# eMWu94/ReMo3D

Measured on AMD Instinct MI355X. Metric: measurement points/sec (3D benchmark model), higher is better.
Workload: dtype f64

## Files before the change

include/remo3d_hip_debug.h:

```cpp
#ifndef REMO3D_HIP_DEBUG_H
#define REMO3D_HIP_DEBUG_H

#include "remo3d_hip.h"

#ifdef __cplusplus
extern "C" {
#endif

int remo_debug_stream(remo_ctx_t *ctx, int64_t bytes, double *read_gbs, double *copy_gbs);
int remo_debug_clock(remo_ctx_t *ctx, double *gfma_per_wave);
int remo_debug_cache_gather(remo_ctx_t *ctx, int64_t bytes, double *gbs);
int remo_debug_device(remo_ctx_t *ctx, int64_t *out8);
int remo_debug_xcc(remo_ctx_t *ctx, int32_t *out, int32_t nblocks);


int remo_debug_patch_phases(remo_ctx_t *ctx, remo_batch_t *batch, int32_t fp32 , double *out16);

int remo_debug_patch_phases_p(remo_ctx_t *ctx, remo_batch_t *batch, int32_t fp32, double *out16);

int remo_debug_grid_barrier(remo_ctx_t *ctx, int32_t nblocks, int32_t nbar, double *out3);

int remo_debug_sens_timing(remo_ctx_t *ctx, double *out2);
int remo_debug_sens_group_timing(remo_ctx_t *ctx, double *out4);
int remo_debug_field_timing(remo_ctx_t *ctx, double *out2);
int remo_debug_point_location(remo_ctx_t *ctx);
int remo_debug_direction_bytes(remo_ctx_t *ctx);
int remo_debug_direction_forms(remo_ctx_t *ctx, int64_t n, int64_t nv, int32_t k, int32_t grid, int32_t step, double tol2, const double *r,
                               const float *p, const double *z, const double *dinv, const double *part_even, const double *part_odd,
                               int32_t nb_rz, const double *scal48, float *p_flat, float *p_row, double *scal_flat, double *scal_row);
int remo_debug_product(remo_ctx_t *ctx, int32_t slots, int64_t cap, int64_t nx, const int32_t *xrp, const int32_t *xc, const double *xv,
                       int64_t ny, const int32_t *yrp, const int32_t *yc, const double *yv, int32_t *crp, int32_t *cc, double *cv,
                       int32_t *flags);
int remo_debug_vector_heads(remo_ctx_t *ctx, int32_t on, double *out8);
int remo_debug_secondary_timing(remo_ctx_t *ctx, double *ms);
int remo_debug_pairs_timing(remo_ctx_t *ctx, double *out2);
int remo_debug_pair_groups_timing(remo_ctx_t *ctx, double *out4);

int remo_debug_tune(int32_t key, int32_t value);

#ifdef __cplusplus
}
#endif
#endif
```

remo3d_amd/_lib.py:

```python
from __future__ import annotations

import ctypes as C
import os

import numpy as np

_HERE = os.path.dirname(os.path.abspath(__file__))
LIB_PATH = os.environ.get("REMO_LIB") or os.path.join(_HERE, "libremo3d_hip.so")
REMO_MAX_RHS = 8


class RemoMesh(C.Structure):
    _fields_ = [("dim", C.c_int32), ("n_nodes", C.c_int64), ("coords", C.POINTER(C.c_double)),
                ("n_elems", C.c_int64), ("conn", C.POINTER(C.c_int32)), ("mat", C.POINTER(C.c_int32)),
                ("n_bfacets", C.c_int64), ("bconn", C.POINTER(C.c_int32)), ("bdirichlet", C.POINTER(C.c_uint8))]


class RemoOpts(C.Structure):
    _fields_ = [("preconditioner", C.c_int32), ("condense", C.c_int32), ("maxsteps", C.c_int32),
                ("check_every", C.c_int32), ("rtol", C.c_double), ("time_kernels", C.c_int32),
                ("coarse_degree", C.c_int32), ("coarse_ratio", C.c_int32), ("precision", C.c_int32), ("inner_digits", C.c_int32),
                ("serialize_solves", C.c_int32), ("op", C.c_int32), ("coarse", C.c_int32), ("assemble", C.c_int32), ("quadrature", C.c_int32)]


class RemoStats(C.Structure):
    _fields_ = [("n_dof", C.c_int64), ("n_free", C.c_int64), ("nnz", C.c_int64), ("n_edges", C.c_int64),
                ("n_faces", C.c_int64), ("n_rhs", C.c_int32), ("max_iterations", C.c_int32),
                ("iterations", C.c_int32 * REMO_MAX_RHS), ("relres", C.c_double * REMO_MAX_RHS),
                ("ms_symbolic", C.c_double), ("ms_h2d", C.c_double), ("ms_assemble", C.c_double),
                ("ms_solve", C.c_double), ("ms_eval", C.c_double), ("ms_total", C.c_double),
                ("spmv_ms", C.c_double), ("spmv_launches", C.c_int64), ("spmv_bytes", C.c_double),
                ("pcg_steps", C.c_int64), ("spmv_ms_raw", C.c_double), ("event_overhead_ms", C.c_double),
                ("refinement_cycles", C.c_int64), ("op_used", C.c_int32), ("coarse_used", C.c_int32),
                ("assembled", C.c_int32), ("patch_rounds", C.c_int32)]

    def as_dict(self):
        d = {}
        for name, _ in self._fields_:
            v = getattr(self, name)
            d[name] = list(v) if hasattr(v, "__len__") else v
        return d


class RemoJob(C.Structure):
    _dp, _ip = C.POINTER(C.c_double), C.POINTER(C.c_int32)
    _fields_ = [("size", C.c_uint32), ("tensor", C.c_int32), ("n_mat", C.c_int32), ("sigma", _dp),
                ("n_rhs", C.c_int32), ("src_ptr", _ip), ("src_p", _dp), ("src_I", _dp),
                ("eval_ptr", _ip), ("eval_p", _dp), ("u_out", _dp),
                ("n_fun", C.c_int32), ("fun_rhs", _ip), ("fun_ptr", _ip), ("fun_p", _dp), ("fun_w", _dp), ("J_out", _dp), ("dJ_out", _dp),
                ("n_group", C.c_int32), ("group", _ip), ("dJg_out", _dp),
                ("warm", C.c_void_p),
                ("n_pts", C.c_int32), ("pts", _dp), ("n_frhs", C.c_int32), ("field_rhs", _ip), ("u_f", _dp), ("grad_f", _dp), ("J_f", _dp),
                ("elem_f", _ip)]


class RemoJobSecondary(C.Structure):
    _fields_ = RemoJob._fields_ + [("secondary", C.c_int32), ("sec_quad", C.c_int32), ("sec_radius", C.c_double),
                                   ("sec_sigma0", C.POINTER(C.c_double))]


class RemoJobError(C.Structure):
    _fields_ = RemoJobSecondary._fields_ + [("err", C.c_int32), ("err_n_group", C.c_int32), ("err_group", C.POINTER(C.c_int32)),
                                            ("err_out", C.POINTER(C.c_double)), ("errg_out", C.POINTER(C.c_double))]


class RemoJobPairs(C.Structure):
    _fields_ = RemoJobError._fields_ + [("n_pair", C.c_int32), ("pair_reserved", C.c_int32), ("pair_a", C.POINTER(C.c_int32)),
                                        ("pair_b", C.POINTER(C.c_int32)), ("dP_out", C.POINTER(C.c_double))]


class RemoJobPairGroups(C.Structure):
    _fields_ = RemoJobPairs._fields_ + [("pair_n_group", C.c_int32), ("pair_group_reserved", C.c_int32), ("pair_group", C.POINTER(C.c_int32)),
                                        ("dPg_out", C.POINTER(C.c_double))]


EXPORTS = ["remo_abi_version", "remo_opts_default", "remo_ctx_create", "remo_ctx_destroy", "remo_last_error",
           "remo_solve_batch", "remo_solve_batch_tensor", "remo_solve_batch_sens", "remo_solve_batch_sens_tensor", "remo_solve_batch_sens_groups", "remo_solve_batch_sens_groups_tensor",
           "remo_solve_batch_field", "remo_solve_batch_field_tensor", "remo_batch_field", "remo_host_field_element",
           "remo_warm_create", "remo_warm_destroy", "remo_warm_clear", "remo_warm_info", "remo_solve_batch_sens_warm", "remo_solve_batch_sens_warm_tensor", "remo_batch_create", "remo_batch_create_tensor", "remo_batch_run", "remo_batch_fetch", "remo_batch_destroy",
           "remo_batch_eval", "remo_batch_get_system", "remo_batch_get_vectors", "remo_batch_apply_coarse", "remo_batch_spmv",
           "remo_host_element_matrix", "remo_host_element_matrix_tensor", "remo_host_sens_element", "remo_host_factor_error", "remo_host_symbolic",
           "remo_solve_job", "remo_batch_create_job", "remo_host_point_shapes", "remo_host_secondary_element", "remo_host_error_facet", "remo_host_pair_element"]
DEBUG_EXPORTS = ["remo_debug_stream", "remo_debug_clock", "remo_debug_device", "remo_debug_cache_gather", "remo_debug_xcc", "remo_debug_tune", "remo_debug_patch_phases", "remo_debug_patch_phases_p", "remo_debug_grid_barrier", "remo_debug_sens_timing", "remo_debug_sens_group_timing", "remo_debug_field_timing", "remo_debug_point_location", "remo_debug_secondary_timing", "remo_debug_direction_bytes", "remo_debug_pairs_timing", "remo_debug_pair_groups_timing",
                 "remo_debug_direction_forms", "remo_debug_vector_heads", "remo_debug_product"]

JOB_HEAD = ["n_mat", "sigma", "n_rhs", "src_ptr", "src_p", "src_I", "eval_ptr", "eval_p"]
_SENS = ["u_out", "n_fun", "fun_rhs", "fun_ptr", "fun_p", "fun_w"]
LEGACY_MEMBERS = {"": ["u_out"],
                  "_sens": _SENS + ["J_out", "dJ_out"],
                  "_sens_warm": _SENS + ["J_out", "dJ_out", "warm"],
                  "_sens_groups": _SENS + ["n_group", "group", "J_out", "dJ_out", "dJg_out"],
                  "_field": ["u_out", "n_pts", "pts", "n_frhs", "field_rhs", "u_f", "grad_f", "J_f", "elem_f"]}


def legacy_args(job, kind=None):
    return [getattr(job, name) for name in JOB_HEAD + (LEGACY_MEMBERS[kind] if kind is not None else [])]


_lib = None


def load():
    global _lib
    if _lib is not None:
        return _lib
    if not os.path.exists(LIB_PATH):
        raise ImportError(f"{LIB_PATH} is missing: build it with `make -C remo3d_amd/csrc` "
                          "(or __graft_entry__.build()); remo3d_amd has no CPU fallback")
    L = C.CDLL(LIB_PATH)
    dp, ip, i64p, u8p = C.POINTER(C.c_double), C.POINTER(C.c_int32), C.POINTER(C.c_int64), C.POINTER(C.c_uint8)
    vp = C.c_void_p
    L.remo_abi_version.restype = C.c_int
    L.remo_opts_default.argtypes = [C.POINTER(RemoOpts)]
    L.remo_ctx_create.restype = vp
    L.remo_ctx_create.argtypes = [C.c_int]
    L.remo_ctx_destroy.argtypes = [vp]
    L.remo_last_error.restype = C.c_char_p
    L.remo_last_error.argtypes = [vp]
    member = dict(RemoJob._fields_)
    batch_args = [vp, C.POINTER(RemoMesh)] + [member[name] for name in JOB_HEAD]
    for kind, names in LEGACY_MEMBERS.items():
        for entry in (getattr(L, "remo_solve_batch" + kind), getattr(L, "remo_solve_batch" + kind + "_tensor")):
            entry.restype = C.c_int
            entry.argtypes = batch_args + [member[name] for name in names] + [C.POINTER(RemoOpts), C.POINTER(RemoStats)]
    L.remo_warm_create.restype = vp
    L.remo_warm_create.argtypes = [C.c_int]
    L.remo_warm_destroy.restype = None
    L.remo_warm_destroy.argtypes = [vp]
    L.remo_warm_clear.restype = None
    L.remo_warm_clear.argtypes = [vp]
    L.remo_warm_info.restype = C.c_int
    L.remo_warm_info.argtypes = [vp, i64p, ip, i64p, ip]
    L.remo_solve_job.restype = C.c_int
    L.remo_solve_job.argtypes = [vp, C.POINTER(RemoMesh), vp, C.POINTER(RemoOpts), C.POINTER(RemoStats)]
    L.remo_batch_create_job.restype = C.c_int
    L.remo_batch_create_job.argtypes = [vp, C.POINTER(RemoMesh), vp, C.POINTER(vp)]
    L.remo_host_point_shapes.restype = C.c_int
    L.remo_host_point_shapes.argtypes = [C.c_int32, dp, dp, dp]
    L.remo_batch_field.restype = C.c_int
    L.remo_batch_field.argtypes = [vp, vp, C.c_int32, C.c_int32, dp, dp, dp, dp, ip]
    L.remo_host_field_element.restype = C.c_int
    L.remo_host_field_element.argtypes = [C.c_int32, dp, dp, C.c_double, dp, dp, dp]
    L.remo_debug_field_timing.restype = C.c_int
    L.remo_debug_field_timing.argtypes = [vp, dp]
    L.remo_debug_point_location.restype = C.c_int
    L.remo_debug_point_location.argtypes = [vp]
    L.remo_debug_direction_bytes.restype = C.c_int
    L.remo_debug_direction_bytes.argtypes = [vp]
    L.remo_host_secondary_element.restype = C.c_int
    L.remo_host_secondary_element.argtypes = [C.c_int32, dp, dp, C.c_double, C.c_double, C.c_double, dp, C.c_int32, dp]
    L.remo_host_error_facet.restype = C.c_int
    L.remo_host_error_facet.argtypes = [C.c_int32, C.c_int32, dp, dp, C.c_double, dp, dp, dp, C.c_double, dp, dp]
    L.remo_debug_secondary_timing.restype = C.c_int
    L.remo_debug_secondary_timing.argtypes = [vp, dp]
    L.remo_debug_sens_group_timing.restype = C.c_int
    L.remo_debug_sens_group_timing.argtypes = [vp, dp]
    L.remo_host_pair_element.restype = C.c_int
    L.remo_host_pair_element.argtypes = [C.c_int32, dp, C.c_int32, C.c_int32, dp, C.c_int32, ip, ip, dp]
    L.remo_debug_pairs_timing.restype = C.c_int
    L.remo_debug_pairs_timing.argtypes = [vp, dp]
    L.remo_debug_pair_groups_timing.restype = C.c_int
    L.remo_debug_pair_groups_timing.argtypes = [vp, dp]
    L.remo_host_sens_element.restype = C.c_int
    L.remo_host_sens_element.argtypes = [C.c_int32, dp, C.c_int32, dp, dp, dp]
    L.remo_debug_sens_timing.restype = C.c_int
    L.remo_debug_sens_timing.argtypes = [vp, dp]
    L.remo_batch_create.restype = C.c_int
    L.remo_batch_create.argtypes = batch_args + [C.POINTER(vp)]
    L.remo_batch_create_tensor.restype = C.c_int
    L.remo_batch_create_tensor.argtypes = batch_args + [C.POINTER(vp)]
    L.remo_batch_run.restype = C.c_int
    L.remo_batch_run.argtypes = [vp, vp, C.POINTER(RemoOpts), C.POINTER(RemoStats)]
    L.remo_batch_fetch.restype = C.c_int
    L.remo_batch_fetch.argtypes = [vp, vp, dp]
    L.remo_batch_destroy.argtypes = [vp, vp]
    L.remo_batch_eval.restype = C.c_int
    L.remo_batch_eval.argtypes = [vp, vp, C.c_int32, C.c_int32, dp, dp]
    L.remo_batch_get_system.restype = C.c_int
    L.remo_batch_get_system.argtypes = [vp, vp, ip, ip, dp, dp, ip]
    L.remo_batch_get_vectors.restype = C.c_int
    L.remo_batch_get_vectors.argtypes = [vp, vp, dp, dp, ip]
    L.remo_batch_apply_coarse.restype = C.c_int
    L.remo_batch_apply_coarse.argtypes = [vp, vp, C.c_int32, dp, dp, C.c_int32, i64p]
    L.remo_debug_patch_phases.restype = C.c_int
    L.remo_debug_patch_phases.argtypes = [vp, vp, C.c_int32, dp]
    L.remo_debug_patch_phases_p.restype = C.c_int
    L.remo_debug_patch_phases_p.argtypes = [vp, vp, C.c_int32, dp]
    L.remo_debug_grid_barrier.restype = C.c_int
    L.remo_debug_grid_barrier.argtypes = [vp, C.c_int32, C.c_int32, dp]
    L.remo_debug_xcc.restype = C.c_int
    L.remo_debug_xcc.argtypes = [vp, ip, C.c_int32]
    L.remo_debug_cache_gather.restype = C.c_int
    L.remo_debug_cache_gather.argtypes = [vp, C.c_int64, dp]
    L.remo_debug_device.restype = C.c_int
    L.remo_debug_device.argtypes = [vp, i64p]
    L.remo_debug_clock.restype = C.c_int
    L.remo_debug_clock.argtypes = [vp, dp]
    L.remo_debug_stream.restype = C.c_int
    L.remo_debug_stream.argtypes = [vp, C.c_int64, dp, dp]
    L.remo_batch_spmv.restype = C.c_int
    L.remo_batch_spmv.argtypes = [vp, vp, C.c_int32, dp, dp, C.c_int32, dp]
    L.remo_host_element_matrix.restype = C.c_int
    L.remo_host_element_matrix.argtypes = [C.c_int32, dp, C.c_double, dp]
    L.remo_host_element_matrix_tensor.restype = C.c_int
    L.remo_host_element_matrix_tensor.argtypes = [C.c_int32, dp, dp, dp]
    L.remo_host_factor_error.restype = C.c_double
    L.remo_host_symbolic.restype = C.c_int
    L.remo_host_symbolic.argtypes = [C.POINTER(RemoMesh), C.c_int32, i64p, ip, ip, ip]
    L.remo_debug_tune.restype = C.c_int
    L.remo_debug_tune.argtypes = [C.c_int32, C.c_int32]
    fp = C.POINTER(C.c_float)
    if hasattr(L, "remo_debug_direction_forms"):
        L.remo_debug_direction_forms.restype = C.c_int
        L.remo_debug_direction_forms.argtypes = [vp, C.c_int64, C.c_int64, C.c_int32, C.c_int32, C.c_int32, C.c_double, dp, fp, dp, dp, dp, dp,
                                                 C.c_int32, dp, fp, fp, dp, dp]
        L.remo_debug_vector_heads.restype = C.c_int
        L.remo_debug_vector_heads.argtypes = [vp, C.c_int32, dp]
    if hasattr(L, "remo_debug_product"):
        L.remo_debug_product.restype = C.c_int
        L.remo_debug_product.argtypes = [vp, C.c_int32, C.c_int64, C.c_int64, ip, ip, dp, C.c_int64, ip, ip, dp, ip, ip, dp, ip]
    _lib = L
    return L


def ptr(a, t):
    return a.ctypes.data_as(C.POINTER(t))


def mesh_struct(mesh):
    coords = np.ascontiguousarray(mesh.coords, dtype=np.float64)
    conn = np.ascontiguousarray(mesh.conn, dtype=np.int32)
    mat = np.ascontiguousarray(mesh.mat, dtype=np.int32)
    bconn = np.ascontiguousarray(mesh.bconn, dtype=np.int32).reshape(-1, mesh.dim)
    bdir = np.ascontiguousarray(mesh.bdirichlet, dtype=np.uint8)
    m = RemoMesh(int(mesh.dim), coords.shape[0], ptr(coords, C.c_double), conn.shape[0], ptr(conn, C.c_int32),
                 ptr(mat, C.c_int32), bconn.shape[0], ptr(bconn, C.c_int32), ptr(bdir, C.c_uint8))
    return m, (coords, conn, mat, bconn, bdir)
```

remo3d_amd/csrc/amg.h:

```cpp
#pragma once
#include <hip/hip_runtime.h>
#include <stdint.h>

#include <string>

#include "symbolic_gpu.h"

namespace remo {

constexpr int kAmgMaxLevels = 8;
constexpr int kAmgDenseMax = 64;

template <class T> struct AmgLevelT {
    int64_t n = 0, nnz = 0, nnz_p = 0;
    const int32_t *rowptr = nullptr, *col = nullptr;
    const T *val = nullptr, *dinv = nullptr;
    const int32_t *p_rowptr = nullptr, *p_col = nullptr;
    const T *p_val = nullptr;
    const int32_t *r_rowptr = nullptr, *r_col = nullptr;
    const T *r_val = nullptr;
    double omega = 0.0;
    T *r = nullptr, *z = nullptr, *z2 = nullptr, *t = nullptr;
};

template <class T> struct AmgT {
    int levels = 0;
    AmgLevelT<T> lev[kAmgMaxLevels];
    const T *inv = nullptr;
    int launches = 0;
    int kmax = 0;
};

bool amg_setup(Arena &ar, hipStream_t s, int dim, int64_t nv, const int32_t *rowptr, const int32_t *col, const double *val, int kmax,
               AmgT<double> &out, std::string &why);
void amg_to_float(Arena &ar, hipStream_t s, const AmgT<double> &in, int kmax, AmgT<float> &out);

void amg_debug_product(hipStream_t s, int slots, int64_t cap, int64_t nx, const int32_t *xrp, const int32_t *xc, const double *xv, int64_t ny,
                       const int32_t *yrp, const int32_t *yc, const double *yv, int32_t *crp, int32_t *cc, double *cv, int32_t *flags);

template <class T, class TR> void launch_amg_cycle(const AmgT<T> &H, int k, int step, const TR *r, TR *cz, double *part, int nblocks, const double *scal,
                                                   hipStream_t s);

}
```

remo3d_amd/csrc/amg.hip:

```cpp
#include <hip/hip_runtime.h>
#include <limits.h>

#include <rocprim/device/device_scan.hpp>

#include <atomic>
#include <cmath>
#include <cstdio>
#include <cstdlib>
#include <cstring>
#include <stdexcept>
#include <string>
#include <vector>

#include "amg.h"
#include "remo_internal.h"
#include "wave_util.h"
#include "kutil.h"

namespace remo {
namespace {

__device__ __forceinline__ void wave_sync() {
    __builtin_amdgcn_fence(__ATOMIC_ACQ_REL, "wavefront");
    __builtin_amdgcn_wave_barrier();
}

__device__ __forceinline__ bool amg_done(const double *scal, int step) {
    if (!scal) return false;
    const int d = reinterpret_cast<const int *>(scal + kDoneSlot)[0];
    return d != 0 && d <= step;
}

template <int PASS>
__global__ void __launch_bounds__(256) k_block_copy(int64_t nv, const int32_t *__restrict__ rowptr, const int32_t *__restrict__ col,
                                                    const double *__restrict__ val, int32_t *__restrict__ cnt, const int32_t *__restrict__ orp,
                                                    int32_t *__restrict__ oc, double *__restrict__ ov) {
    const int64_t row = int64_t(blockIdx.x) * blockDim.x + threadIdx.x;
    if (row >= nv) return;
    const int32_t rs = rowptr[row], re = rowptr[row + 1];
    if (PASS == 0) {
        cnt[row] = lower_bound_i32(col, rs, re, int32_t(nv)) - rs;
    } else {
        const int32_t at = orp[row], len = orp[row + 1] - at;
        for (int32_t e = 0; e < len; ++e) { oc[at + e] = col[rs + e]; ov[at + e] = val[rs + e]; }
    }
}

__global__ void __launch_bounds__(256) k_level_diag(int64_t n, const int32_t *__restrict__ rowptr, const int32_t *__restrict__ col,
                                                    const double *__restrict__ val, double *__restrict__ dinv, unsigned long long *bound_bits,
                                                    int32_t *flag) {
    double m = 0.0;
    const int64_t row = int64_t(blockIdx.x) * blockDim.x + threadIdx.x;
    if (row < n) {
        double s = 0.0, d = 0.0;
        for (int32_t p = rowptr[row]; p < rowptr[row + 1]; ++p) {
            s += fabs(val[p]);
            if (col[p] == row) d = val[p];
        }
        if (!(d > 0.0)) { atomicOr(flag, 1); d = 1.0; }
        dinv[row] = 1.0 / d;
        m = s / d;
    }
#pragma unroll
    for (int off = 32; off > 0; off >>= 1) m = fmax(m, __shfl_xor(m, off, 64));
    if ((threadIdx.x & 63) == 0) atomicMax(bound_bits, (unsigned long long)__double_as_longlong(m));
}

constexpr uint64_t kTupMask = (uint64_t(1) << 62) - 1;

__device__ __forceinline__ uint32_t hash_u32(uint32_t x) {
    x ^= x >> 16; x *= 0x7feb352du; x ^= x >> 15; x *= 0x846ca68bu; x ^= x >> 16;
    return x;
}

__global__ void __launch_bounds__(256) k_mis_init(int64_t n, uint64_t *__restrict__ tup) {
    const int64_t i = int64_t(blockIdx.x) * blockDim.x + threadIdx.x;
    if (i < n) tup[i] = (uint64_t(1) << 62) | (uint64_t(hash_u32(uint32_t(i)) >> 2) << 32) | uint64_t(uint32_t(i));
}

__global__ void __launch_bounds__(256) k_mis_max(int64_t n, const int32_t *__restrict__ rowptr, const int32_t *__restrict__ col,
                                                 const uint64_t *__restrict__ tup, uint64_t *__restrict__ m1) {
    const int64_t i = int64_t(blockIdx.x) * blockDim.x + threadIdx.x;
    if (i >= n) return;
    uint64_t m = tup[i];
    for (int32_t p = rowptr[i]; p < rowptr[i + 1]; ++p) { const uint64_t t = tup[col[p]]; m = t > m ? t : m; }
    m1[i] = m;
}

__global__ void __launch_bounds__(256) k_mis_update(int64_t n, const int32_t *__restrict__ rowptr, const int32_t *__restrict__ col,
                                                    uint64_t *__restrict__ tup, const uint64_t *__restrict__ m1) {
    const int64_t i = int64_t(blockIdx.x) * blockDim.x + threadIdx.x;
    if (i >= n) return;
    const uint64_t t = tup[i];
    if ((t >> 62) != 1) return;
    uint64_t m = m1[i];
    for (int32_t p = rowptr[i]; p < rowptr[i + 1]; ++p) { const uint64_t v = m1[col[p]]; m = v > m ? v : m; }
    if (m == t) tup[i] = (uint64_t(2) << 62) | (t & kTupMask);
    else if ((m >> 62) == 2) tup[i] = t & kTupMask;
}

__global__ void __launch_bounds__(256) k_mis_finish(int64_t n, const int32_t *__restrict__ rowptr, const int32_t *__restrict__ col,
                                                    const uint64_t *__restrict__ tup, uint64_t *__restrict__ out) {
    const int64_t i = int64_t(blockIdx.x) * blockDim.x + threadIdx.x;
    if (i >= n) return;
    const uint64_t t = tup[i];
    uint64_t r = t;
    if ((t >> 62) == 1) {
        bool top = true;
        for (int32_t p = rowptr[i]; p < rowptr[i + 1]; ++p) {
            const uint64_t v = tup[col[p]];
            if ((v >> 62) == 1 && v > t) top = false;
        }
        r = top ? ((uint64_t(2) << 62) | (t & kTupMask)) : (t & kTupMask);
    }
    out[i] = r;
}

__global__ void __launch_bounds__(256) k_mis_flags(int64_t n, const uint64_t *__restrict__ tup, int32_t *__restrict__ isroot) {
    const int64_t i = int64_t(blockIdx.x) * blockDim.x + threadIdx.x;
    if (i < n) isroot[i] = (tup[i] >> 62) == 2 ? 1 : 0;
}

__global__ void __launch_bounds__(256) k_agg_near(int64_t n, const int32_t *__restrict__ rowptr, const int32_t *__restrict__ col,
                                                  const uint64_t *__restrict__ tup, const int32_t *__restrict__ id, int32_t *__restrict__ agg) {
    const int64_t i = int64_t(blockIdx.x) * blockDim.x + threadIdx.x;
    if (i >= n) return;
    if ((tup[i] >> 62) == 2) { agg[i] = id[i]; return; }
    uint64_t best = 0;
    int32_t bj = -1;
    for (int32_t p = rowptr[i]; p < rowptr[i + 1]; ++p) {
        const int32_t j = col[p];
        const uint64_t t = tup[j];
        if ((t >> 62) == 2 && t > best) { best = t; bj = j; }
    }
    agg[i] = bj >= 0 ? id[bj] : -1;
}

__global__ void __launch_bounds__(256) k_agg_far(int64_t n, const int32_t *__restrict__ rowptr, const int32_t *__restrict__ col,
                                                 const double *__restrict__ val, const int32_t *__restrict__ agg_in, int32_t *__restrict__ agg_out) {
    const int64_t i = int64_t(blockIdx.x) * blockDim.x + threadIdx.x;
    if (i >= n) return;
    int32_t a = agg_in[i];
    if (a < 0) {
        double w = -1.0;
        for (int32_t p = rowptr[i]; p < rowptr[i + 1]; ++p) {
            const int32_t j = col[p];
            if (j == i) continue;
            const int32_t aj = agg_in[j];
            const double v = fabs(val[p]);
            if (aj >= 0 && v > w) { w = v; a = aj; }
        }
    }
    agg_out[i] = a;
}

__global__ void __launch_bounds__(256) k_smoothing_factor(int64_t n, const int32_t *__restrict__ rowptr, const int32_t *__restrict__ col,
                                                          const double *__restrict__ val, const double *__restrict__ dinv, const unsigned long long *bound_bits,
                                                          double *__restrict__ sval, const int32_t *__restrict__ agg, int32_t *__restrict__ p0rp,
                                                          int32_t *__restrict__ p0c, double *__restrict__ p0v) {
    const int64_t i = int64_t(blockIdx.x) * blockDim.x + threadIdx.x;
    if (i > n) return;
    p0rp[i] = int32_t(i);
    if (i == n) return;
    const double f = 4.0 / (3.0 * __longlong_as_double((long long)bound_bits[0])) * dinv[i];
    for (int32_t p = rowptr[i]; p < rowptr[i + 1]; ++p) sval[p] = (col[p] == i ? 1.0 : 0.0) - f * val[p];
    const int32_t a = agg[i];
    p0c[i] = a >= 0 ? a : 0;
    p0v[i] = a >= 0 ? 1.0 : 0.0;
}

template <int PASS, int SLOTS>
__global__ void __launch_bounds__(256) k_spgemm(int64_t nx, const int32_t *__restrict__ xrp, const int32_t *__restrict__ xc, const double *__restrict__ xv,
                                                const int32_t *__restrict__ yrp, const int32_t *__restrict__ yc, const double *__restrict__ yv,
                                                int32_t *__restrict__ cnt, const int32_t *__restrict__ crp, int32_t *__restrict__ cc,
                                                double *__restrict__ cv, int32_t *flag) {
    __shared__ int32_t keys[4][SLOTS];
    __shared__ int32_t list[4][SLOTS];
    constexpr int kTerms = SLOTS < 512 ? 512 : 1024;
    __shared__ double terms[4][PASS == 1 ? kTerms : 1];
    __shared__ int32_t pstart[4][PASS == 1 ? 64 : 1], pys[4][PASS == 1 ? 64 : 1];
    __shared__ double pxv[4][PASS == 1 ? 64 : 1];
    const int wave = threadIdx.x >> 6, lane = threadIdx.x & 63;
    const int64_t row = int64_t(blockIdx.x) * 4 + wave;
    if (row >= nx) return;
    int32_t *K = keys[wave], *L = list[wave];
    for (int sl = lane; sl < SLOTS; sl += 64) K[sl] = INT_MAX;
    wave_sync();
    const int32_t xs = xrp[row], xe = xrp[row + 1];
    bool overflow = false;
    for (int32_t p = xs + lane; p < xe; p += 64) {
        const int32_t k = xc[p];
        const int32_t ye = yrp[k + 1];
        for (int32_t q = yrp[k]; q < ye; ++q) {
            const int32_t j = yc[q];
            uint32_t h = ((uint32_t(j) * 2654435761u) >> 16) & (SLOTS - 1);
            bool placed = false;
            for (int probe = 0; probe < SLOTS; ++probe) {
                const int32_t old = atomicCAS(&K[h], INT_MAX, j);
                if (old == INT_MAX || old == j) { placed = true; break; }
                h = (h + 1) & (SLOTS - 1);
            }
            overflow |= !placed;
        }
    }
    wave_sync();
    int c = 0;
    for (int base = 0; base < SLOTS; base += 64) {
        const int32_t v = K[base + lane];
        const bool occ = v != INT_MAX;
        const uint64_t bal = __builtin_amdgcn_ballot_w64(occ);
        if (occ) L[c + __builtin_popcountll(bal & ((uint64_t(1) << lane) - 1))] = v;
        c += __builtin_popcountll(bal);
    }
    if (__builtin_amdgcn_ballot_w64(overflow) != 0 || c > SLOTS / 2) {
        if (lane == 0) atomicOr(flag, 1);
        c = 0;
    }
    if (PASS == 0) {
        if (lane == 0) cnt[row] = c;
        return;
    }
    if (c == 0) return;
    int m = 64;
    while (m < c) m <<= 1;
    for (int t = c + lane; t < m; t += 64) L[t] = INT_MAX;
    wave_sync();
    for (int size = 2; size <= m; size <<= 1)
        for (int stride = size >> 1; stride > 0; stride >>= 1) {
            for (int t = lane; t < m / 2; t += 64) {
                const int lo = 2 * t - (t & (stride - 1));
                const int hi = lo + stride;
                const bool up = (lo & size) == 0;
                const int32_t a = L[lo], b = L[hi];
                if ((a > b) == up) { L[lo] = b; L[hi] = a; }
            }
            wave_sync();
        }
    const int64_t off = crp[row];
    const int room = int(crp[row + 1] - crp[row]);
    if (c > room) c = room;
    if (c <= 0) return;
    double *V = terms[wave];
    int32_t *PS = pstart[wave], *PY = pys[wave];
    double *PX = pxv[wave];
    constexpr int NACC = SLOTS / 128;
    double acc[NACC];
#pragma unroll
    for (int a = 0; a < NACC; ++a) acc[a] = 0.0;
    const int npmax = kTerms / c < 64 ? kTerms / c : 64;
    for (int i = lane; i < c * npmax; i += 64) V[i] = 0.0;
    for (int32_t p0 = xs; p0 < xe; p0 += npmax) {
        const int np = (xe - p0 < npmax) ? int(xe - p0) : npmax;
        int32_t ys = 0, len = 0;
        double xval = 0.0;
        if (lane < np) {
            const int32_t k = xc[p0 + lane];
            xval = xv[p0 + lane];
            ys = yrp[k];
            len = yrp[k + 1] - ys;
        }
        int32_t incl = len;
#pragma unroll
        for (int off = 1; off < 64; off <<= 1) {
            const int32_t up = __shfl_up(incl, off, 64);
            if (lane >= off) incl += up;
        }
        const int32_t total = __shfl(incl, 63, 64);
        if (lane < np) { PS[lane] = incl - len; PY[lane] = ys; PX[lane] = xval; }
        wave_sync();
        for (int32_t idx = lane; idx < total; idx += 64) {
            int lo = 1, hi = np;
            while (lo < hi) {
                const int mid = (lo + hi) >> 1;
                if (PS[mid] <= idx) lo = mid + 1; else hi = mid;
            }
            const int pp = lo - 1;
            const int32_t q = PY[pp] + (idx - PS[pp]);
            const int32_t j = yc[q];
            const double yval = yv[q];
            const int t = lower_bound_i32(L, 0, c, j);
            if (t < c && L[t] == j) V[pp * c + t] = PX[pp] * yval;
        }
        wave_sync();
#pragma unroll
        for (int a = 0; a < NACC; ++a) {
            const int t = lane + 64 * a;
            if (t < c)
                for (int pp = 0; pp < np; ++pp) { acc[a] += V[pp * c + t]; V[pp * c + t] = 0.0; }
        }
    }
#pragma unroll
    for (int a = 0; a < NACC; ++a) {
        const int t = lane + 64 * a;
        if (t < c) { cc[off + t] = L[t]; cv[off + t] = acc[a]; }
    }
}

__global__ void __launch_bounds__(256) k_clamp_rowptr(int64_t n, int32_t *__restrict__ rowptr, int32_t capacity, int32_t *flag) {
    const int64_t i = int64_t(blockIdx.x) * blockDim.x + threadIdx.x;
    if (i > n) return;
    const int32_t v = rowptr[i];
    if (v > capacity) { rowptr[i] = capacity; if (i == n) atomicOr(flag, 2); }
}

__global__ void __launch_bounds__(256) k_tr_count(int64_t n, const int32_t *__restrict__ rowptr, const int32_t *__restrict__ col, int32_t *__restrict__ cnt) {
    const int64_t i = int64_t(blockIdx.x) * blockDim.x + threadIdx.x;
    if (i >= n) return;
    for (int32_t p = rowptr[i]; p < rowptr[i + 1]; ++p) atomicAdd(&cnt[col[p]], 1);
}
__global__ void __launch_bounds__(256) k_tr_fill(int64_t n, const int32_t *__restrict__ rowptr, const int32_t *__restrict__ col, const double *__restrict__ val,
                                                 const int32_t *__restrict__ rrp, int32_t *__restrict__ cursor, int32_t *__restrict__ rc, double *__restrict__ rv) {
    const int64_t i = int64_t(blockIdx.x) * blockDim.x + threadIdx.x;
    if (i >= n) return;
    for (int32_t p = rowptr[i]; p < rowptr[i + 1]; ++p) {
        const int32_t c = col[p];
        const int32_t at = rrp[c] + atomicAdd(&cursor[c], 1);
        rc[at] = int32_t(i);
        rv[at] = val[p];
    }
}
constexpr int kTrMax = 512, kTrMaxLong = 4096;
template <int MINLEN, int MAXLEN, int WAVES>
__global__ void __launch_bounds__(64 * WAVES) k_tr_sort(int64_t nr, const int32_t *__restrict__ rrp, int32_t *__restrict__ rc, double *__restrict__ rv, int32_t *flag) {
    __shared__ int32_t keys[WAVES][MAXLEN];
    __shared__ double vals[WAVES][MAXLEN];
    const int wave = threadIdx.x >> 6, lane = threadIdx.x & 63;
    const int64_t row = int64_t(blockIdx.x) * WAVES + wave;
    if (row >= nr) return;
    const int32_t rs = rrp[row], len = rrp[row + 1] - rs;
    if (len <= 1 || len <= MINLEN) return;
    if (len > MAXLEN) { if (lane == 0 && MAXLEN == kTrMaxLong) atomicOr(flag, 4); return; }
    int32_t *K = keys[wave];
    double *V = vals[wave];
    int m = 64;
    while (m < len) m <<= 1;
    for (int t = lane; t < m; t += 64) { K[t] = t < len ? rc[rs + t] : INT_MAX; V[t] = t < len ? rv[rs + t] : 0.0; }
    wave_sync();
    for (int size = 2; size <= m; size <<= 1)
        for (int stride = size >> 1; stride > 0; stride >>= 1) {
            for (int t = lane; t < m / 2; t += 64) {
                const int lo = 2 * t - (t & (stride - 1));
                const int hi = lo + stride;
                const bool up = (lo & size) == 0;
                const int32_t a = K[lo], b = K[hi];
                if ((a > b) == up) { K[lo] = b; K[hi] = a; const double x = V[lo]; V[lo] = V[hi]; V[hi] = x; }
            }
            wave_sync();
        }
    for (int t = lane; t < len; t += 64) { rc[rs + t] = K[t]; rv[rs + t] = V[t]; }
}

__global__ void __launch_bounds__(256) k_dense_inverse(int n, const int32_t *__restrict__ rowptr, const int32_t *__restrict__ col,
                                                       const double *__restrict__ val, double *__restrict__ inv, int32_t *flag) {
    __shared__ double a[kAmgDenseMax * kAmgDenseMax];
    const int tid = threadIdx.x;
    for (int e = tid; e < n * n; e += 256) a[e] = 0.0;
    __syncthreads();
    for (int i = tid; i < n; i += 256)
        for (int32_t p = rowptr[i]; p < rowptr[i + 1]; ++p) a[i * n + col[p]] = val[p];
    __syncthreads();
    for (int p = 0; p < n; ++p) {
        const double piv = a[p * n + p];
        if (!(piv > 0.0)) { if (tid == 0) atomicOr(flag, 2); return; }
        const double ip = 1.0 / piv;
        __syncthreads();
        for (int j = tid; j < n; j += 256)
            if (j != p) a[p * n + j] *= ip;
        __syncthreads();
        for (int e = tid; e < n * n; e += 256) {
            const int i = e / n, j = e - i * n;
            if (i != p && j != p) a[e] -= a[i * n + p] * a[p * n + j];
        }
        __syncthreads();
        for (int i = tid; i < n; i += 256)
            a[i * n + p] = (i == p) ? ip : -a[i * n + p] * ip;
        __syncthreads();
    }
    for (int e = tid; e < n * n; e += 256) inv[e] = a[e];
}

template <class S, class D> __global__ void __launch_bounds__(256) k_convert(int64_t n, const S *__restrict__ src, D *__restrict__ dst) {
    const int64_t i = int64_t(blockIdx.x) * blockDim.x + threadIdx.x;
    if (i < n) dst[i] = D(src[i]);
}

constexpr int kLpr = 8;

template <class T, int K, bool SCALE, int LPR = kLpr, class TX = T>
__device__ __forceinline__ void row_product(int32_t rs, int32_t re, int sub, const int32_t *__restrict__ col, const T *__restrict__ val,
                                            const T *__restrict__ dinv, const TX *__restrict__ x, T (&acc)[K]) {
#pragma unroll
    for (int c = 0; c < K; ++c) acc[c] = T(0);
    for (int32_t p0 = rs + sub; p0 < re; p0 += 2 * LPR) {
        int32_t j[2];
        T a[2], xv[2][K];
#pragma unroll
        for (int u = 0; u < 2; ++u) {
            const int32_t p = p0 + u * LPR;
            j[u] = -1; a[u] = T(0);
            if (p < re) { j[u] = col[p]; a[u] = val[p]; }
        }
#pragma unroll
        for (int u = 0; u < 2; ++u) {
#pragma unroll
            for (int c = 0; c < K; ++c) xv[u][c] = T(0);
            if (j[u] >= 0) {
                if (SCALE) a[u] *= dinv[j[u]];
                const TX *xr = x + int64_t(j[u]) * K;
#pragma unroll
                for (int c = 0; c < K; ++c) xv[u][c] = T(xr[c]);
            }
        }
#pragma unroll
        for (int u = 0; u < 2; ++u)
#pragma unroll
            for (int c = 0; c < K; ++c) acc[c] += a[u] * xv[u][c];
    }
    TReduce<K, LPR>::run(acc, sub);
}

struct Lane {
    int sub, mycol;
    bool mine;
};
template <int K, int LPR = kLpr> __device__ __forceinline__ Lane lane_of(int tid) {
    int idx[K], own[K];
    Lane l;
    l.sub = tid % LPR;
    towner_init<K, LPR>(idx, own, l.sub);
    l.mycol = idx[0];
    l.mine = own[0] != 0;
    return l;
}

template <class T, int K, class TR = T> __device__ __forceinline__ void op_pre(const AmgLevelT<T> &a, const TR *__restrict__ r, int64_t row, const Lane &ln) {
    T acc[K];
    row_product<T, K, true, kLpr, TR>(a.rowptr[row], a.rowptr[row + 1], ln.sub, a.col, a.val, a.dinv, r, acc);
    if (ln.mine) {
        const int64_t at = row * K + ln.mycol;
        const T w = T(a.omega), ri = T(r[at]);
        a.z[at] = w * a.dinv[row] * ri;
        a.t[at] = ri - w * acc[0];
    }
}
template <class T, int K, int LPR = kLpr> __device__ __forceinline__ void op_restrict(const AmgLevelT<T> &a, T *__restrict__ rn, int64_t row, const Lane &ln) {
    T acc[K];
    row_product<T, K, false, LPR>(a.r_rowptr[row], a.r_rowptr[row + 1], ln.sub, a.r_col, a.r_val, (const T *)nullptr, (const T *)a.t, acc);
    if (ln.mine) rn[row * K + ln.mycol] = acc[0];
}
template <class T, int K> __device__ __forceinline__ void op_prolong(const AmgLevelT<T> &a, const T *__restrict__ zn, int64_t row, const Lane &ln) {
    T acc[K];
    row_product<T, K, false>(a.p_rowptr[row], a.p_rowptr[row + 1], ln.sub, a.p_col, a.p_val, (const T *)nullptr, zn, acc);
    if (ln.mine) a.z[row * K + ln.mycol] += acc[0];
}
template <class T, int K, bool LAST, class TR = T>
__device__ __forceinline__ double op_post(const AmgLevelT<T> &a, const TR *__restrict__ r, TR *__restrict__ zout, int64_t row, const Lane &ln) {
    T acc[K];
    row_product<T, K, false>(a.rowptr[row], a.rowptr[row + 1], ln.sub, a.col, a.val, (const T *)nullptr, (const T *)a.z, acc);
    double dot = 0.0;
    if (ln.mine) {
        const int64_t at = row * K + ln.mycol;
        const TR rr = r[at];
        const T ri = T(rr), di = a.dinv[row];
        const T zn = a.z[at] + T(a.omega) * di * (ri - acc[0]);
        zout[at] = TR(LAST ? zn / di : zn);
        dot = double(rr) * double(zn);
    }
    return dot;
}

constexpr int kRpb = 256 / kLpr;

template <class T, int K, class TR>
__global__ void __launch_bounds__(256) k_amg_pre(AmgLevelT<T> a, const TR *__restrict__ r, const double *scal, int step) {
    if (amg_done(scal, step)) return;
    const Lane ln = lane_of<K>(threadIdx.x);
    const int64_t row = int64_t(blockIdx.x) * kRpb + threadIdx.x / kLpr;
    if (row < a.n) op_pre<T, K, TR>(a, r, row, ln);
}
template <class T, int K>
__global__ void __launch_bounds__(256) k_amg_restrict(AmgLevelT<T> a, int64_t n_next, T *__restrict__ rn, const double *scal, int step) {
    if (amg_done(scal, step)) return;
    const Lane ln = lane_of<K>(threadIdx.x);
    const int64_t row = int64_t(blockIdx.x) * kRpb + threadIdx.x / kLpr;
    if (row < n_next) op_restrict<T, K>(a, rn, row, ln);
}
template <class T, int K>
__global__ void __launch_bounds__(256) k_amg_prolong(AmgLevelT<T> a, const T *__restrict__ zn, const double *scal, int step) {
    if (amg_done(scal, step)) return;
    const Lane ln = lane_of<K>(threadIdx.x);
    const int64_t row = int64_t(blockIdx.x) * kRpb + threadIdx.x / kLpr;
    if (row < a.n) op_prolong<T, K>(a, zn, row, ln);
}
template <class T, int K, bool LAST, int THREADS, class TR>
__global__ void __launch_bounds__(THREADS) k_amg_post(AmgLevelT<T> a, const TR *__restrict__ r, TR *__restrict__ zout,
                                                     double *__restrict__ part, const double *scal, int step) {
    if (amg_done(scal, step)) return;
    const Lane ln = lane_of<K>(threadIdx.x);
    constexpr int RPB = THREADS / kLpr;
    double dot = 0.0;
    for (int64_t row = int64_t(blockIdx.x) * RPB + threadIdx.x / kLpr; row < a.n; row += int64_t(gridDim.x) * RPB)
        dot += op_post<T, K, LAST, TR>(a, r, zout, row, ln);
    if (LAST) {
        constexpr int NW = THREADS / 64;
        __shared__ double smem[NW * K];
        const int lane = threadIdx.x & 63, wave = threadIdx.x >> 6;
#pragma unroll
        for (int k = 0; k < K; ++k) {
            const double x = wave_sum((ln.mine && k == ln.mycol) ? dot : 0.0);
            if (lane == 0) smem[wave * K + k] = x;
        }
        __syncthreads();
        if (threadIdx.x < K) {
            double t = 0.0;
            for (int w = 0; w < NW; ++w) t += smem[w * K + threadIdx.x];
            part[blockIdx.x * K + threadIdx.x] = t;
        }
    }
}

template <class T, int K>
__device__ __forceinline__ void op_dense(int n, const T *__restrict__ inv, const T *__restrict__ r, T *__restrict__ z, int t) {
    const int row = t / K, c = t - row * K;
    T acc = T(0);
    for (int j = 0; j < n; ++j) acc += inv[j * n + row] * r[j * K + c];
    z[t] = acc;
}

constexpr int kTailLevels = 3;
constexpr int kTailRows = 128;
template <class T> struct AmgTailT {
    int levels;
    AmgLevelT<T> up;
    AmgLevelT<T> lev[kTailLevels];
    const T *inv;
};
template <class T, int K>
__global__ void __launch_bounds__(1024) k_amg_tail(AmgTailT<T> A, const double *scal, int step) {
    if (amg_done(scal, step)) return;
    const Lane ln = lane_of<K>(threadIdx.x);
    const int g = threadIdx.x / kLpr, ng = 1024 / kLpr;
    const int L = A.levels;
    {
        const Lane l16 = lane_of<K, 16>(threadIdx.x);
        for (int64_t row = threadIdx.x / 16; row < A.lev[0].n; row += 1024 / 16) op_restrict<T, K, 16>(A.up, A.lev[0].r, row, l16);
        __syncthreads();
    }
    for (int l = 0; l + 1 < L; ++l) {
        const AmgLevelT<T> &a = A.lev[l];
        for (int64_t row = g; row < a.n; row += ng) op_pre<T, K>(a, (const T *)a.r, row, ln);
        __syncthreads();
        const AmgLevelT<T> &b = A.lev[l + 1];
        for (int64_t row = g; row < b.n; row += ng) op_restrict<T, K>(a, b.r, row, ln);
        __syncthreads();
    }
    {
        const AmgLevelT<T> &c = A.lev[L - 1];
        for (int t = threadIdx.x; t < int(c.n) * K; t += 1024) op_dense<T, K>(int(c.n), A.inv, (const T *)c.r, c.z2, t);
        __syncthreads();
    }
    for (int l = L - 2; l >= 0; --l) {
        const AmgLevelT<T> &a = A.lev[l];
        const AmgLevelT<T> &b = A.lev[l + 1];
        for (int64_t row = g; row < a.n; row += ng) op_prolong<T, K>(a, (const T *)b.z2, row, ln);
        __syncthreads();
        for (int64_t row = g; row < a.n; row += ng) (void)op_post<T, K, false>(a, (const T *)a.r, a.z2, row, ln);
        __syncthreads();
    }
}

int grid_rows(int64_t n, int per_block) { return int((n + per_block - 1) / per_block); }

void scan_counts(Arena &ar, hipStream_t s, int64_t n, const int32_t *cnt, int32_t *out) {
    size_t tb = 0;
    HIP_TRY(rocprim::exclusive_scan(nullptr, tb, cnt, out, int32_t(0), size_t(n + 1), rocprim::plus<int32_t>(), s));
    void *tmp = ar.hi<char>(tb + 256);
    HIP_TRY(rocprim::exclusive_scan(tmp, tb, cnt, out, int32_t(0), size_t(n + 1), rocprim::plus<int32_t>(), s));
}

struct Csr {
    int64_t n = 0, nnz = 0;
    int32_t *rowptr = nullptr, *col = nullptr;
    double *val = nullptr;
};

template <int PASS>
void launch_product(int variant, hipStream_t s, const Csr &X, const Csr &Y, int32_t *cnt, const int32_t *crp, int32_t *cc, double *cv, int32_t *d_over) {
    if (variant <= 1)
        hipLaunchKernelGGL((k_spgemm<PASS, 128>), dim3(grid_rows(X.n, 4)), dim3(256), 0, s, X.n, X.rowptr, X.col, X.val, Y.rowptr, Y.col, Y.val, cnt, crp, cc, cv, d_over);
    else
        hipLaunchKernelGGL((k_spgemm<PASS, 512>), dim3(grid_rows(X.n, 4)), dim3(256), 0, s, X.n, X.rowptr, X.col, X.val, Y.rowptr, Y.col, Y.val, cnt, crp, cc, cv, d_over);
}

void spgemm_async(Arena &ar, bool permanent, hipStream_t s, const Csr &X, const Csr &Y, int64_t cap, int variant, int32_t *d_over, Csr &C) {
    if (cap > INT_MAX - 8) cap = INT_MAX - 8;
    C.n = X.n;
    C.nnz = cap;
    C.rowptr = permanent ? ar.lo<int32_t>(size_t(X.n) + 2) : ar.hi<int32_t>(size_t(X.n) + 2);
    int32_t *cnt = ar.hi<int32_t>(size_t(X.n) + 2);
    launch_product<0>(variant, s, X, Y, cnt, nullptr, nullptr, nullptr, d_over);
    scan_counts(ar, s, X.n, cnt, C.rowptr);
    hipLaunchKernelGGL(k_clamp_rowptr, dim3(grid_rows(X.n + 1, 256)), dim3(256), 0, s, X.n, C.rowptr, int32_t(cap), d_over);
    C.col = permanent ? ar.lo<int32_t>(size_t(cap) + 2) : ar.hi<int32_t>(size_t(cap) + 2);
    C.val = permanent ? ar.lo<double>(size_t(cap) + 2) : ar.hi<double>(size_t(cap) + 2);
    launch_product<1>(variant, s, X, Y, nullptr, C.rowptr, C.col, C.val, d_over);
}

std::atomic<int> g_product_hint[2][kAmgMaxLevels][3];
std::atomic<int> g_ap_room[2];
constexpr int kFlagSlots = 64;

int amg_build(Arena &ar, hipStream_t s, int hs, int64_t nv, const int32_t *rowptr, const int32_t *col, const double *val, int kmax, AmgT<double> &H,
              std::string &why) {
    H = AmgT<double>{};
    int32_t *d_flag = ar.lo<int32_t>(kFlagSlots);
    unsigned long long *d_bound = ar.lo<unsigned long long>(kAmgMaxLevels + 1);
    HIP_TRY(hipMemsetAsync(d_flag, 0, sizeof(int32_t) * kFlagSlots, s));
    HIP_TRY(hipMemsetAsync(d_bound, 0, sizeof(unsigned long long) * (kAmgMaxLevels + 1), s));
    int32_t h_flags[kFlagSlots] = {};
    int32_t h_nnz_a[kAmgMaxLevels] = {}, h_nnz_p[kAmgMaxLevels] = {};
    const int32_t *d_nnz_p[kAmgMaxLevels] = {};
    auto check = [&](int upto) -> int {
        int again = 0;
        for (int l = 0; l < upto; ++l)
            for (int p = 0; p < 3; ++p) {
                const int f = h_flags[8 + 3 * l + p];
                if (f == 0) continue;
                if (f & 1) {
                    if (g_product_hint[hs][l][p].load() >= 2) { why = "a product row with more than 256 distinct columns"; return -1; }
                    g_product_hint[hs][l][p].store(2);
                    again = 1;
                }
                if (f & 2) {
                    if (p != 1 || g_ap_room[hs].load() >= 3) { why = "a product outgrew its arrays"; return -1; }
                    g_ap_room[hs].fetch_add(1);
                    again = 1;
                }
            }
        if (again) return 1;
        if (h_flags[0] != 0) {
            why = "setup raised flag " + std::to_string(h_flags[0]) + " (1 diagonal, 2 dense pivot, 4 a row of R beyond the LDS sort)";
            return -1;
        }
        return 0;
    };
    Csr A;
    A.n = nv;
    A.rowptr = ar.lo<int32_t>(size_t(nv) + 2);
    {
        const size_t mark = ar.hi_mark();
        int32_t *cnt = ar.hi<int32_t>(size_t(nv) + 2);
        hipLaunchKernelGGL((k_block_copy<0>), dim3(grid_rows(nv, 256)), dim3(256), 0, s, nv, rowptr, col, val, cnt, (const int32_t *)nullptr,
                           (int32_t *)nullptr, (double *)nullptr);
        scan_counts(ar, s, nv, cnt, A.rowptr);
        int32_t h = 0;
        HIP_TRY(hipMemcpyAsync(&h, A.rowptr + nv, sizeof(int32_t), hipMemcpyDeviceToHost, s));
        HIP_TRY(hipStreamSynchronize(s));
        ar.hi_release(mark);
        if (h <= 0 || h == INT_MAX) { why = "empty vertex block"; return -1; }
        A.nnz = h;
        h_nnz_a[0] = h;
        A.col = ar.lo<int32_t>(size_t(h) + 2);
        A.val = ar.lo<double>(size_t(h) + 2);
        hipLaunchKernelGGL((k_block_copy<1>), dim3(grid_rows(nv, 256)), dim3(256), 0, s, nv, rowptr, col, val, (int32_t *)nullptr,
                           (const int32_t *)A.rowptr, A.col, A.val);
    }
    int L = 0;
    for (;;) {
        AmgLevelT<double> &lv = H.lev[L];
        const int64_t n = A.n;
        lv.n = n; lv.rowptr = A.rowptr; lv.col = A.col; lv.val = A.val;
        double *dinv = ar.lo<double>(size_t(n) + 2);
        lv.dinv = dinv;
        lv.z = ar.lo<double>(size_t(n) * kmax + 2);
        lv.z2 = ar.lo<double>(size_t(n) * kmax + 2);
        lv.t = ar.lo<double>(size_t(n) * kmax + 2);
        if (L > 0) lv.r = ar.lo<double>(size_t(n) * kmax + 2);
        const int g = grid_rows(n, 256);
        hipLaunchKernelGGL(k_level_diag, dim3(g), dim3(256), 0, s, n, A.rowptr, A.col, A.val, dinv, d_bound + L, d_flag);
        if (n <= kAmgDenseMax) {
            double *inv = ar.lo<double>(size_t(n) * n + 2);
            hipLaunchKernelGGL(k_dense_inverse, dim3(1), dim3(256), 0, s, int(n), A.rowptr, A.col, A.val, inv, d_flag);
            H.inv = inv;
            H.levels = L + 1;
            break;
        }
        if (L + 1 >= kAmgMaxLevels) { why = "too many levels"; return -1; }
        const size_t mark = ar.hi_mark();
        uint64_t *tup = ar.hi<uint64_t>(size_t(n) + 2), *m1 = ar.hi<uint64_t>(size_t(n) + 2);
        int32_t *isroot = ar.hi<int32_t>(size_t(n) + 2), *id = ar.hi<int32_t>(size_t(n) + 2);
        int32_t *agg1 = ar.hi<int32_t>(size_t(n) + 2), *agg = ar.hi<int32_t>(size_t(n) + 2);
        hipLaunchKernelGGL(k_mis_init, dim3(g), dim3(256), 0, s, n, tup);
        for (int it = 0; it < 10; ++it) {
            hipLaunchKernelGGL(k_mis_max, dim3(g), dim3(256), 0, s, n, A.rowptr, A.col, tup, m1);
            hipLaunchKernelGGL(k_mis_update, dim3(g), dim3(256), 0, s, n, A.rowptr, A.col, tup, m1);
        }
        hipLaunchKernelGGL(k_mis_finish, dim3(g), dim3(256), 0, s, n, A.rowptr, A.col, tup, m1);
        hipLaunchKernelGGL(k_mis_flags, dim3(g), dim3(256), 0, s, n, m1, isroot);
        scan_counts(ar, s, n, isroot, id);
        hipLaunchKernelGGL(k_agg_near, dim3(g), dim3(256), 0, s, n, A.rowptr, A.col, m1, id, agg1);
        hipLaunchKernelGGL(k_agg_far, dim3(g), dim3(256), 0, s, n, A.rowptr, A.col, A.val, agg1, agg);
        int32_t h_nc = 0;
        unsigned long long h_bound = 0;
        HIP_TRY(hipMemcpyAsync(&h_nc, id + n, sizeof(int32_t), hipMemcpyDeviceToHost, s));
        HIP_TRY(hipMemcpyAsync(&h_bound, d_bound + L, sizeof(unsigned long long), hipMemcpyDeviceToHost, s));
        HIP_TRY(hipMemcpyAsync(h_flags, d_flag, sizeof(int32_t) * kFlagSlots, hipMemcpyDeviceToHost, s));
        if (L > 0) HIP_TRY(hipMemcpyAsync(&h_nnz_a[L], A.rowptr + n, sizeof(int32_t), hipMemcpyDeviceToHost, s));
        HIP_TRY(hipStreamSynchronize(s));
        const int verdict = check(L);
        if (verdict != 0) return verdict;
        double lmax;
        std::memcpy(&lmax, &h_bound, sizeof lmax);
        const int64_t nnz_a = h_nnz_a[L];
        if (getenv("REMO_AMG_DEBUG")) fprintf(stderr, "amg level %d: n %lld nnz %lld -> %d aggregates, lmax %.3f\n", L, (long long)n, (long long)nnz_a, h_nc, lmax);
        if (!(lmax > 0.0) || !std::isfinite(lmax) || nnz_a <= 0) { why = "level operator without a spectrum bound"; return -1; }
        lv.omega = 1.6 / lmax;
        lv.nnz = nnz_a;
        const int64_t nc = h_nc;
        if (nc <= 0 || nc * 10 > n * 8) { why = "no coarsening"; return -1; }
        Csr S = A, P0;
        S.val = ar.hi<double>(size_t(nnz_a) + 2);
        P0.n = n; P0.nnz = n;
        P0.rowptr = ar.hi<int32_t>(size_t(n) + 2); P0.col = ar.hi<int32_t>(size_t(n) + 2); P0.val = ar.hi<double>(size_t(n) + 2);
        hipLaunchKernelGGL(k_smoothing_factor, dim3(grid_rows(n + 1, 256)), dim3(256), 0, s, n, A.rowptr, A.col, A.val, dinv, d_bound + L, S.val,
                           agg, P0.rowptr, P0.col, P0.val);
        int32_t *pf = d_flag + 8 + 3 * L;
        Csr P;
        spgemm_async(ar, true, s, S, P0, nnz_a, g_product_hint[hs][L][0].load(), pf + 0, P);
        lv.p_rowptr = P.rowptr; lv.p_col = P.col; lv.p_val = P.val;
        d_nnz_p[L] = P.rowptr + n;
        Csr R;
        R.n = nc; R.nnz = nnz_a;
        R.rowptr = ar.lo<int32_t>(size_t(nc) + 2); R.col = ar.lo<int32_t>(size_t(nnz_a) + 2); R.val = ar.lo<double>(size_t(nnz_a) + 2);
        {
            int32_t *tcnt = ar.hi<int32_t>(size_t(nc) + 2), *cursor = ar.hi<int32_t>(size_t(nc) + 2);
            HIP_TRY(hipMemsetAsync(tcnt, 0, sizeof(int32_t) * (size_t(nc) + 2), s));
            HIP_TRY(hipMemsetAsync(cursor, 0, sizeof(int32_t) * (size_t(nc) + 2), s));
            hipLaunchKernelGGL(k_tr_count, dim3(g), dim3(256), 0, s, n, P.rowptr, P.col, tcnt);
            scan_counts(ar, s, nc, tcnt, R.rowptr);
            hipLaunchKernelGGL(k_tr_fill, dim3(g), dim3(256), 0, s, n, P.rowptr, P.col, P.val, R.rowptr, cursor, R.col, R.val);
            hipLaunchKernelGGL((k_tr_sort<0, kTrMax, 4>), dim3(grid_rows(nc, 4)), dim3(256), 0, s, nc, R.rowptr, R.col, R.val, d_flag);
            hipLaunchKernelGGL((k_tr_sort<kTrMax, kTrMaxLong, 1>), dim3(grid_rows(nc, 1)), dim3(64), 0, s, nc, R.rowptr, R.col, R.val, d_flag);
        }
        lv.r_rowptr = R.rowptr; lv.r_col = R.col; lv.r_val = R.val;
        Csr AP, Ac;
        spgemm_async(ar, false, s, A, P, (nnz_a * 4) << g_ap_room[hs].load(), g_product_hint[hs][L][1].load(), pf + 1, AP);
        spgemm_async(ar, true, s, R, AP, nnz_a, g_product_hint[hs][L][2].load(), pf + 2, Ac);
        ar.hi_release(mark);
        A = Ac;
        A.n = nc;
        ++L;
    }
    HIP_TRY(hipMemcpyAsync(h_flags, d_flag, sizeof(int32_t) * kFlagSlots, hipMemcpyDeviceToHost, s));
    HIP_TRY(hipMemcpyAsync(&h_nnz_a[L], A.rowptr + A.n, sizeof(int32_t), hipMemcpyDeviceToHost, s));
    for (int l = 0; l < L; ++l) HIP_TRY(hipMemcpyAsync(&h_nnz_p[l], d_nnz_p[l], sizeof(int32_t), hipMemcpyDeviceToHost, s));
    HIP_TRY(hipStreamSynchronize(s));
    const int verdict = check(L);
    if (verdict != 0) return verdict;
    H.lev[L].nnz = h_nnz_a[L];
    for (int l = 0; l < L; ++l) H.lev[l].nnz_p = h_nnz_p[l];
    H.launches = 4 * (H.levels - 1);
    H.kmax = kmax;
    return 0;
}

}

bool amg_setup(Arena &ar, hipStream_t s, int dim, int64_t nv, const int32_t *rowptr, const int32_t *col, const double *val, int kmax, AmgT<double> &H,
               std::string &why) {
    H = AmgT<double>{};
    if (nv <= kAmgDenseMax) { why = "vertex block too small"; return false; }
    const int hs = dim == 3 ? 1 : 0;
    const size_t hi0 = ar.hi_mark(), lo0 = ar.lo_off;
    try {
        for (int attempt = 0; attempt < 6; ++attempt) {
            ar.hi_release(hi0);
            ar.lo_off = lo0;
            const int rc = amg_build(ar, s, hs, nv, rowptr, col, val, kmax, H, why);
            ar.hi_release(hi0);
            if (rc == 0) return true;
            if (rc < 0) break;
        }
        if (why.empty()) why = "the products did not fit after several attempts";
        H = AmgT<double>{};
        ar.lo_off = lo0;
        return false;
    } catch (const std::exception &ex) {
        ar.hi_release(hi0);
        ar.lo_off = lo0;
        H = AmgT<double>{};
        why = ex.what();
        return false;
    }
}

void amg_debug_product(hipStream_t s, int slots, int64_t cap, int64_t nx, const int32_t *xrp, const int32_t *xc, const double *xv, int64_t ny,
                       const int32_t *yrp, const int32_t *yc, const double *yv, int32_t *crp, int32_t *cc, double *cv, int32_t *flags) {
    if (slots != 128 && slots != 512) throw std::runtime_error("amg_debug_product: 128 or 512 slots");
    if (nx < 1 || ny < 1 || nx > (1 << 24) || ny > (1 << 24) || cap < 1 || cap > (1 << 28)) throw std::runtime_error("amg_debug_product: sizes out of range");
    auto ascending = [](const int32_t *rp, int64_t n) {
        if (rp[0] != 0) return false;
        for (int64_t i = 0; i < n; ++i)
            if (rp[i + 1] < rp[i]) return false;
        return rp[n] <= (1 << 28);
    };
    if (!ascending(xrp, nx) || !ascending(yrp, ny)) throw std::runtime_error("amg_debug_product: row pointers must ascend from 0");
    const size_t nnzx = size_t(xrp[nx]), nnzy = size_t(yrp[ny]);
    for (size_t p = 0; p < nnzx; ++p)
        if (xc[p] < 0 || xc[p] >= ny) throw std::runtime_error("amg_debug_product: a column of X names no row of Y");
    for (size_t q = 0; q < nnzy; ++q)
        if (yc[q] < 0 || yc[q] == INT_MAX) throw std::runtime_error("amg_debug_product: a column of Y out of range");
    const size_t ints = 2 * (size_t(nx) + size_t(ny) + 4) + nnzx + nnzy + 2 * size_t(nx) + size_t(cap) + 16 + kFlagSlots;
    const size_t bytes = 4 * ints + 8 * (nnzx + nnzy + size_t(cap) + 8) + 16 * size_t(nx) + (size_t(1) << 20);
    DeviceTemp tmp;
    Arena ar;
    ar.base = tmp.alloc<char>(bytes);
    ar.cap = bytes;
    HIP_TRY(hipMemsetAsync(ar.base, 0xFF, bytes, s));
    Csr X, Y, C;
    auto put = [&](Csr &M, int64_t n, size_t nnz, const int32_t *rp, const int32_t *c, const double *v) {
        M.n = n; M.nnz = int64_t(nnz);
        M.rowptr = ar.lo<int32_t>(size_t(n) + 2); M.col = ar.lo<int32_t>(nnz + 2); M.val = ar.lo<double>(nnz + 2);
        HIP_TRY(hipMemcpyAsync(M.rowptr, rp, sizeof(int32_t) * (size_t(n) + 1), hipMemcpyHostToDevice, s));
        if (nnz) {
            HIP_TRY(hipMemcpyAsync(M.col, c, sizeof(int32_t) * nnz, hipMemcpyHostToDevice, s));
            HIP_TRY(hipMemcpyAsync(M.val, v, sizeof(double) * nnz, hipMemcpyHostToDevice, s));
        }
    };
    put(X, nx, nnzx, xrp, xc, xv);
    put(Y, ny, nnzy, yrp, yc, yv);
    int32_t *d_flag = ar.lo<int32_t>(kFlagSlots);
    HIP_TRY(hipMemsetAsync(d_flag, 0, sizeof(int32_t) * kFlagSlots, s));
    spgemm_async(ar, true, s, X, Y, cap, slots == 128 ? 1 : 2, d_flag, C);
    HIP_TRY(hipGetLastError());
    HIP_TRY(hipMemcpyAsync(crp, C.rowptr, sizeof(int32_t) * (size_t(nx) + 1), hipMemcpyDeviceToHost, s));
    HIP_TRY(hipMemcpyAsync(cc, C.col, sizeof(int32_t) * (size_t(cap) + 2), hipMemcpyDeviceToHost, s));
    HIP_TRY(hipMemcpyAsync(cv, C.val, sizeof(double) * (size_t(cap) + 2), hipMemcpyDeviceToHost, s));
    HIP_TRY(hipMemcpyAsync(flags, d_flag, sizeof(int32_t), hipMemcpyDeviceToHost, s));
    HIP_TRY(hipStreamSynchronize(s));
}

void amg_to_float(Arena &ar, hipStream_t s, const AmgT<double> &in, int kmax, AmgT<float> &out) {
    auto conv = [&](const double *src, size_t count) {
        float *dst = ar.lo<float>(count + 4);
        hipLaunchKernelGGL((k_convert<double, float>), dim3(grid_rows(int64_t(count), 256)), dim3(256), 0, s, int64_t(count), src, dst);
        return (const float *)dst;
    };
    out = AmgT<float>{};
    out.levels = in.levels;
    out.launches = in.launches;
    out.kmax = kmax;
    for (int l = 0; l < in.levels; ++l) {
        const AmgLevelT<double> &a = in.lev[l];
        AmgLevelT<float> &b = out.lev[l];
        b.n = a.n; b.nnz = a.nnz; b.rowptr = a.rowptr; b.col = a.col; b.omega = a.omega;
        b.val = conv(a.val, size_t(a.nnz));
        b.dinv = conv(a.dinv, size_t(a.n));
        b.z = ar.lo<float>(size_t(a.n) * kmax + 4); b.z2 = ar.lo<float>(size_t(a.n) * kmax + 4); b.t = ar.lo<float>(size_t(a.n) * kmax + 4);
        if (l > 0) b.r = ar.lo<float>(size_t(a.n) * kmax + 4);
        if (l + 1 < in.levels) {
            b.p_rowptr = a.p_rowptr; b.p_col = a.p_col; b.r_rowptr = a.r_rowptr; b.r_col = a.r_col;
            b.nnz_p = a.nnz_p;
            b.p_val = conv(a.p_val, size_t(a.nnz_p));
            b.r_val = conv(a.r_val, size_t(a.nnz_p));
        }
    }
    const int64_t nc = in.lev[in.levels - 1].n;
    out.inv = conv(in.inv, size_t(nc * nc));
}

template <class T, class TR> void launch_amg_cycle(const AmgT<T> &H, int k, int step, const TR *r, TR *cz, double *part, int nblocks, const double *scal, hipStream_t s) {
    const int L = H.levels;
    auto rows_grid = [&](int64_t n) { return int((n + kRpb - 1) / kRpb); };
    int lt = L - 1;
    while (lt > 1 && H.lev[lt - 1].n <= kTailRows && L - (lt - 1) <= kTailLevels) --lt;
    for_k(k, [&](auto kc) {
        constexpr int K = decltype(kc)::value;
        for (int l = 0; l < lt; ++l) {
            const AmgLevelT<T> &a = H.lev[l], &b = H.lev[l + 1];
            if (l == 0) hipLaunchKernelGGL((k_amg_pre<T, K, TR>), dim3(rows_grid(a.n)), dim3(256), 0, s, a, r, scal, step);
            else hipLaunchKernelGGL((k_amg_pre<T, K, T>), dim3(rows_grid(a.n)), dim3(256), 0, s, a, (const T *)a.r, scal, step);
            if (l + 1 < lt) hipLaunchKernelGGL((k_amg_restrict<T, K>), dim3(rows_grid(b.n)), dim3(256), 0, s, a, b.n, b.r, scal, step);
        }
        {
            AmgTailT<T> tail;
            tail.levels = L - lt;
            tail.up = H.lev[lt - 1];
            for (int l = lt; l < L; ++l) tail.lev[l - lt] = H.lev[l];
            tail.inv = H.inv;
            hipLaunchKernelGGL((k_amg_tail<T, K>), dim3(1), dim3(1024), 0, s, tail, scal, step);
        }
        for (int l = lt - 1; l >= 0; --l) {
            const AmgLevelT<T> &a = H.lev[l], &b = H.lev[l + 1];
            hipLaunchKernelGGL((k_amg_prolong<T, K>), dim3(rows_grid(a.n)), dim3(256), 0, s, a, (const T *)b.z2, scal, step);
            if (l == 0)
                hipLaunchKernelGGL((k_amg_post<T, K, true, 1024, TR>), dim3(nblocks), dim3(1024), 0, s, a, r, cz, part, scal, step);
            else
                hipLaunchKernelGGL((k_amg_post<T, K, false, 256, T>), dim3(rows_grid(a.n)), dim3(256), 0, s, a, (const T *)a.r, a.z2, (double *)nullptr, scal, step);
        }
    });
}

template void launch_amg_cycle<double, double>(const AmgT<double> &, int, int, const double *, double *, double *, int, const double *, hipStream_t);
template void launch_amg_cycle<float, float>(const AmgT<float> &, int, int, const float *, float *, double *, int, const double *, hipStream_t);
template void launch_amg_cycle<float, double>(const AmgT<float> &, int, int, const double *, double *, double *, int, const double *, hipStream_t);

}
```

remo3d_amd/csrc/remo_debug.hip:

```cpp
#include <limits.h>

#include <algorithm>
#include <vector>

#include "../../include/remo3d_hip_debug.h"
#include "remo_internal.h"
#include "patch.h"

using namespace remo;

namespace remo {
Tune g_tune;
}

extern "C" {

namespace {
__global__ void __launch_bounds__(256) k_stream_read(const double2 *__restrict__ x, int64_t n2, double *__restrict__ out) {
    double a = 0.0, b = 0.0;
    for (int64_t i = int64_t(blockIdx.x) * blockDim.x + threadIdx.x; i < n2; i += int64_t(gridDim.x) * blockDim.x) {
        const double2 v = x[i];
        a += v.x; b += v.y;
    }
    a += b;
    for (int off = 32; off > 0; off >>= 1) a += __shfl_xor(a, off, 64);
    if ((threadIdx.x & 63) == 0) out[blockIdx.x * 4 + (threadIdx.x >> 6)] = a;
}
__global__ void __launch_bounds__(256) k_l2_gather(const double2 *__restrict__ x, uint32_t mask, int iters, double *__restrict__ out) {
    uint32_t idx = (blockIdx.x * 256u + threadIdx.x) * 2654435761u;
    double a = 0.0;
    for (int i = 0; i < iters; ++i) {
        const double2 v = x[idx & mask];
        a += v.x + v.y;
        idx = idx * 1664525u + 1013904223u;
    }
    if (a == 1.2345e300) out[0] = a;
}

__global__ void __launch_bounds__(64) k_clock_probe(int iters, float *__restrict__ out) {
    float a = float(threadIdx.x) * 1e-3f;
    for (int i = 0; i < iters; ++i) {
#pragma unroll
        for (int u = 0; u < 16; ++u) a = __builtin_fmaf(a, 0.999999f, 0.5f);
    }
    if (a == 123.456f) out[blockIdx.x] = a;
}
}

int remo_debug_cache_gather(remo_ctx_t *ctx, int64_t bytes, double *gbs) {
    if (!ctx || !gbs || bytes < (1 << 20) || bytes > (int64_t(1) << 32) || (bytes & (bytes - 1)) != 0) return REMO_ERR_ARG;
    try {
        HIP_TRY(hipSetDevice(ctx->device));
        const int64_t n2 = bytes / 16;
        DeviceTemp tmp;
        double *a = tmp.alloc<double>(size_t(n2) * 2), *o = tmp.alloc<double>(8);
        HIP_TRY(hipMemsetAsync(a, 0, size_t(n2) * 16, ctx->stream));
        const int blocks = 4096, iters = 64;
        float best = 1e30f;
        for (int rep = 0; rep < 5; ++rep) {
            HIP_TRY(hipEventRecord(ctx->ev[0], ctx->stream));
            hipLaunchKernelGGL(k_l2_gather, dim3(blocks), dim3(256), 0, ctx->stream, reinterpret_cast<const double2 *>(a), uint32_t(n2 - 1), iters, o);
            HIP_TRY(hipEventRecord(ctx->ev[1], ctx->stream));
            HIP_TRY(hipStreamSynchronize(ctx->stream));
            float ms = 0;
            (void)hipEventElapsedTime(&ms, ctx->ev[0], ctx->ev[1]);
            if (ms < best) best = ms;
        }
        *gbs = double(blocks) * 256.0 * iters * 16.0 / (double(best) * 1e6);
        return REMO_OK;
    } catch (const std::exception &ex) {
        return fail(ctx, REMO_ERR_DEVICE, ex.what());
    }
}

int remo_debug_clock(remo_ctx_t *ctx, double *gfma_per_wave) {
    if (!ctx || !gfma_per_wave) return REMO_ERR_ARG;
    try {
        HIP_TRY(hipSetDevice(ctx->device));
        DeviceTemp tmp;
        float *o = tmp.alloc<float>(1024);
        const int iters = 1 << 16;
        float best = 1e30f;
        for (int rep = 0; rep < 4; ++rep) {
            HIP_TRY(hipEventRecord(ctx->ev[0], ctx->stream));
            hipLaunchKernelGGL(k_clock_probe, dim3(1024), dim3(64), 0, ctx->stream, iters, o);
            HIP_TRY(hipEventRecord(ctx->ev[1], ctx->stream));
            HIP_TRY(hipStreamSynchronize(ctx->stream));
            float ms = 0;
            (void)hipEventElapsedTime(&ms, ctx->ev[0], ctx->ev[1]);
            if (ms < best) best = ms;
        }
        *gfma_per_wave = double(iters) * 16.0 / (double(best) * 1e6);
        return REMO_OK;
    } catch (const std::exception &ex) {
        return fail(ctx, REMO_ERR_DEVICE, ex.what());
    }
}

namespace {
__global__ void __launch_bounds__(64) k_xcc_probe(int32_t *__restrict__ out) {
    const int32_t id = __builtin_amdgcn_s_getreg((3 << 11) | 20);
    if (threadIdx.x == 0) out[blockIdx.x] = id;
}
}

int remo_debug_xcc(remo_ctx_t *ctx, int32_t *out, int32_t nblocks) {
    if (!ctx || !out || nblocks < 1 || nblocks > 65536) return REMO_ERR_ARG;
    try {
        HIP_TRY(hipSetDevice(ctx->device));
        DeviceTemp tmp;
        int32_t *d = tmp.alloc<int32_t>(nblocks);
        hipLaunchKernelGGL(k_xcc_probe, dim3(nblocks), dim3(64), 0, ctx->stream, d);
        HIP_TRY(hipStreamSynchronize(ctx->stream));
        HIP_TRY(hipMemcpy(out, d, sizeof(int32_t) * nblocks, hipMemcpyDeviceToHost));
        return REMO_OK;
    } catch (const std::exception &ex) {
        return fail(ctx, REMO_ERR_DEVICE, ex.what());
    }
}

int remo_debug_device(remo_ctx_t *ctx, int64_t *out8) {
    if (!ctx || !out8) return REMO_ERR_ARG;
    hipDeviceProp_t pr;
    if (hipGetDeviceProperties(&pr, ctx->device) != hipSuccess) return fail(ctx, REMO_ERR_DEVICE, "hipGetDeviceProperties failed");
    out8[0] = pr.multiProcessorCount;
    out8[1] = pr.clockRate;
    out8[2] = pr.memoryClockRate;
    out8[3] = pr.memoryBusWidth;
    out8[4] = pr.l2CacheSize;
    out8[5] = int64_t(pr.totalGlobalMem >> 20);
    out8[6] = pr.maxSharedMemoryPerMultiProcessor;
    out8[7] = pr.asicRevision;
    return REMO_OK;
}

int remo_debug_stream(remo_ctx_t *ctx, int64_t bytes, double *read_gbs, double *copy_gbs) {
    if (!ctx || bytes < (1 << 20)) return REMO_ERR_ARG;
    try {
        HIP_TRY(hipSetDevice(ctx->device));
        const int64_t n = bytes / 16 * 2;
        DeviceTemp tmp;
        double *a = tmp.alloc<double>(n), *b = tmp.alloc<double>(n), *o = tmp.alloc<double>(4096 * 4);
        HIP_TRY(hipMemsetAsync(a, 0, sizeof(double) * n, ctx->stream));
        HIP_TRY(hipMemsetAsync(b, 0, sizeof(double) * n, ctx->stream));
        float best_r = 1e30f, best_c = 1e30f;
        for (int rep = 0; rep < 6; ++rep) {
            HIP_TRY(hipEventRecord(ctx->ev[0], ctx->stream));
            hipLaunchKernelGGL(k_stream_read, dim3(4096), dim3(256), 0, ctx->stream, reinterpret_cast<const double2 *>(a), n / 2, o);
            HIP_TRY(hipEventRecord(ctx->ev[1], ctx->stream));
            HIP_TRY(hipMemcpyAsync(b, a, sizeof(double) * n, hipMemcpyDeviceToDevice, ctx->stream));
            HIP_TRY(hipEventRecord(ctx->ev[2], ctx->stream));
            HIP_TRY(hipStreamSynchronize(ctx->stream));
            float r = 0, c = 0;
            (void)hipEventElapsedTime(&r, ctx->ev[0], ctx->ev[1]);
            (void)hipEventElapsedTime(&c, ctx->ev[1], ctx->ev[2]);
            if (r < best_r) best_r = r;
            if (c < best_c) best_c = c;
        }
        if (read_gbs) *read_gbs = double(n) * 8.0 / (double(best_r) * 1e6);
        if (copy_gbs) *copy_gbs = 2.0 * double(n) * 8.0 / (double(best_c) * 1e6);
        if (bytes <= (int64_t(192) << 20) && read_gbs) {
            float best = 1e30f;
            for (int rep = 0; rep < 6; ++rep) {
                hipLaunchKernelGGL(k_stream_read, dim3(4096), dim3(256), 0, ctx->stream, reinterpret_cast<const double2 *>(a), n / 2, o);
                HIP_TRY(hipEventRecord(ctx->ev[0], ctx->stream));
                for (int k = 0; k < 4; ++k)
                    hipLaunchKernelGGL(k_stream_read, dim3(4096), dim3(256), 0, ctx->stream, reinterpret_cast<const double2 *>(a), n / 2, o);
                HIP_TRY(hipEventRecord(ctx->ev[1], ctx->stream));
                HIP_TRY(hipStreamSynchronize(ctx->stream));
                float r = 0;
                (void)hipEventElapsedTime(&r, ctx->ev[0], ctx->ev[1]);
                if (r < best) best = r;
            }
            *read_gbs = 4.0 * double(n) * 8.0 / (double(best) * 1e6);
        }
        return REMO_OK;
    } catch (const std::exception &ex) {
        return fail(ctx, REMO_ERR_DEVICE, ex.what());
    }
}

int remo_debug_grid_barrier(remo_ctx_t *ctx, int32_t nblocks, int32_t nbar, double *out3) {
    if (!ctx || !out3 || nblocks < 1 || nblocks > 2048 || nbar < 1 || nbar > 100000) return REMO_ERR_ARG;
    try {
        HIP_TRY(hipSetDevice(ctx->device));
        DeviceTemp tmp;
        unsigned *counter = tmp.alloc<unsigned>(16);
        float *buf = tmp.alloc<float>(size_t(nblocks) * 256);
        int *fail_flag = reinterpret_cast<int *>(counter) + 4, *mismatch = reinterpret_cast<int *>(counter) + 8;
        hipEvent_t e0, e1;
        HIP_TRY(hipEventCreate(&e0)); HIP_TRY(hipEventCreate(&e1));
        float ms = 0.f;
        for (int rep = 0; rep < 2; ++rep) {
            HIP_TRY(hipMemsetAsync(counter, 0, 64, ctx->stream));
            HIP_TRY(hipMemsetAsync(buf, 0, sizeof(float) * size_t(nblocks) * 256, ctx->stream));
            HIP_TRY(hipEventRecord(e0, ctx->stream));
            launch_barrier_probe(nblocks, nbar, counter, fail_flag, buf, mismatch, ctx->stream);
            HIP_TRY(hipEventRecord(e1, ctx->stream));
            HIP_TRY(hipStreamSynchronize(ctx->stream));
            HIP_TRY(hipEventElapsedTime(&ms, e0, e1));
        }
        int h[12];
        HIP_TRY(hipMemcpy(h, counter, sizeof h, hipMemcpyDeviceToHost));
        out3[0] = 1e3 * double(ms) / (2.0 * nbar);
        out3[1] = h[4]; out3[2] = h[8];
        (void)hipEventDestroy(e0); (void)hipEventDestroy(e1);
        return REMO_OK;
    } catch (const std::exception &e) {
        return fail(ctx, REMO_ERR_DEVICE, e.what());
    }
}

#ifdef REMO_PROBES
namespace {
struct PatchProbe {
    static constexpr int k = 5;
    remo_ctx *ctx;
    remo_batch *b;
    bool fp32;
    DeviceTemp tmp;
    double *dx, *dy;
    long long *st;
    size_t stamp_words;
    int nb;
    CsrViewT<float> A32;
    PatchOpT<float> P32;
    PatchProbe(remo_ctx *ctx_, remo_batch *b_, bool fp32_, size_t stamp_words_)
        : ctx(ctx_), b(b_), fp32(fp32_), stamp_words(stamp_words_), A32{b_->A.n, 0, nullptr, nullptr, nullptr}, P32(patch_view32(b_->patch64)) {
        const int64_t n = b->A.n;
        dx = tmp.alloc<double>(n * k + 2);
        dy = tmp.alloc<double>(n * k + 2);
        st = tmp.alloc<long long>(stamp_words);
        std::vector<double> hx(size_t(n) * k);
        for (size_t i = 0; i < hx.size(); ++i) hx[i] = double((i * 2654435761u) % 1000) * 1e-3 - 0.5;
        HIP_TRY(hipMemcpy(dx, hx.data(), sizeof(double) * hx.size(), hipMemcpyHostToDevice));
        HIP_TRY(hipMemset(st, 0, sizeof(long long) * stamp_words));
        nb = spmv_grid(n, choose_lanes_per_row(n, b->A.nnz));
        A32.patch = &P32; A32.vertex_block_only = true;
    }
    void once() {
        if (fp32) launch_spmm(A32, k, reinterpret_cast<const float *>(dx), reinterpret_cast<float *>(dy), nullptr, nullptr, nb, ctx->stream);
        else launch_spmm(b->A, k, dx, dy, nullptr, nullptr, nb, ctx->stream);
    }
    void stamped_runs() {
        set_patch_stamps(st); g_tune.patch_mode = 4;
        for (int rep = 0; rep < 3; ++rep) once();
        g_tune.patch_mode = 0; set_patch_stamps(nullptr);
        HIP_TRY(hipStreamSynchronize(ctx->stream));
    }
    double timed_us() {
        once();
        HIP_TRY(hipEventRecord(ctx->ev[0], ctx->stream));
        for (int rep = 0; rep < 10; ++rep) once();
        HIP_TRY(hipEventRecord(ctx->ev[1], ctx->stream));
        HIP_TRY(hipStreamSynchronize(ctx->stream));
        float ms = 0;
        (void)hipEventElapsedTime(&ms, ctx->ev[0], ctx->ev[1]);
        return 1e3 * double(ms) / 10.0;
    }
    std::vector<long long> stamps() {
        std::vector<long long> h(stamp_words);
        HIP_TRY(hipMemcpy(h.data(), st, sizeof(long long) * h.size(), hipMemcpyDeviceToHost));
        return h;
    }
};

int patch_probe_check(remo_ctx *ctx, remo_batch *b) {
    if (!b->has_system || b->run_id != ctx->run_id || !b->A.patch) return fail(ctx, REMO_ERR_ARG, "the last run on this batch did not use the patch operator");
    if (b->patch64.t.rounds != 1) return fail(ctx, REMO_ERR_ARG, "the batch's patch tables hold two elements per lane: set remo_debug_tune key 40 to 1 and run the batch again");
    if (PatchProbe::k * b->patch64.t.E > kPatchBlock) return fail(ctx, REMO_ERR_ARG, "the batch's patch tables are laid out for fewer than 5 columns");
    return REMO_OK;
}
}
#endif

int remo_debug_patch_phases(remo_ctx_t *ctx, remo_batch_t *b, int32_t fp32, double *out16) {
    if (!ctx || !b || !out16) return REMO_ERR_ARG;
#ifndef REMO_PROBES
    (void)fp32;
    return fail(ctx, REMO_ERR_ARG, "remo_debug_patch_phases: the library was built without -DREMO_PROBES (make -C remo3d_amd/csrc probes)");
#else
    if (int rc = patch_probe_check(ctx, b)) return rc;
    struct PersistOff { int was = g_tune.patch_persist; PersistOff() { g_tune.patch_persist = 0; } ~PersistOff() { g_tune.patch_persist = was; } } persist_off;
    try {
        HIP_TRY(hipSetDevice(ctx->device));
        const int64_t grid = (b->patch64.t.npatch + 7) / 8 * 8;
        std::vector<long long> h;
        {
            PatchProbe pr(ctx, b, fp32 != 0, size_t(grid) * 8);
            pr.stamped_runs();
            for (int mode = 0; mode <= 3; ++mode) {
                g_tune.patch_mode = mode;
                out16[10 + mode] = pr.timed_us();
            }
            g_tune.patch_mode = 0;
            h = pr.stamps();
        }
        for (int i = 0; i < 10; ++i) out16[i] = 0.0;
        long long lo = LLONG_MAX, hi = 0;
        int64_t cnt = 0;
        for (int64_t w = 0; w < grid; ++w) {
            const long long *s8 = h.data() + w * 8;
            if (s8[0] == 0 || s8[7] == 0) continue;
            for (int q = 0; q < 7; ++q) out16[q] += double(s8[q + 1] - s8[q]);
            out16[7] += double(s8[7] - s8[0]);
            lo = std::min(lo, s8[0]); hi = std::max(hi, s8[7]);
            ++cnt;
        }
        for (int q = 0; q < 8; ++q) out16[q] /= double(cnt > 0 ? cnt : 1);
        out16[8] = double(hi - lo);
        out16[9] = double(cnt);
        return REMO_OK;
    } catch (const std::exception &ex) {
        g_tune.patch_mode = 0; set_patch_stamps(nullptr);
        return fail(ctx, REMO_ERR_DEVICE, ex.what());
    }
#endif
}

int remo_debug_patch_phases_p(remo_ctx_t *ctx, remo_batch_t *b, int32_t fp32, double *out16) {
    if (!ctx || !b || !out16) return REMO_ERR_ARG;
#ifndef REMO_PROBES
    (void)fp32;
    return fail(ctx, REMO_ERR_ARG, "remo_debug_patch_phases_p: the library was built without -DREMO_PROBES (make -C remo3d_amd/csrc probes)");
#else
    if (int rc = patch_probe_check(ctx, b)) return rc;
    const int64_t slots = 8192;
    try {
        HIP_TRY(hipSetDevice(ctx->device));
        std::vector<long long> h;
        double us = 0.0;
        {
            PatchProbe pr(ctx, b, fp32 != 0, size_t(slots) * 12);
            pr.stamped_runs();
            us = pr.timed_us();
            h = pr.stamps();
        }
        for (int i = 0; i < 16; ++i) out16[i] = 0.0;
        double patches = 0, wgs = 0, longest = 0;
        for (int64_t w = 0; w < slots; ++w) {
            const long long *s12 = h.data() + w * 12;
            if (s12[10] <= 0) continue;
            double tot = 0;
            for (int q = 0; q < 10; ++q) { out16[q] += double(s12[q]); tot += double(s12[q]); }
            patches += double(s12[10]); wgs += 1; longest = std::max(longest, tot);
        }
        for (int q = 0; q < 10; ++q) out16[q] /= (patches > 0 ? patches : 1);
        out16[10] = patches; out16[11] = wgs; out16[12] = longest; out16[13] = us;
        return REMO_OK;
    } catch (const std::exception &ex) {
        g_tune.patch_mode = 0; set_patch_stamps(nullptr);
        return fail(ctx, REMO_ERR_DEVICE, ex.what());
    }
#endif
}

int remo_debug_direction_forms(remo_ctx_t *ctx, int64_t n, int64_t nv, int32_t k, int32_t grid, int32_t step, double tol2, const double *r,
                               const float *p, const double *z, const double *dinv, const double *part_even, const double *part_odd,
                               int32_t nb_rz, const double *scal48, float *p_flat, float *p_row, double *scal_flat, double *scal_row) {
    if (!ctx || n < 1 || nv < 0 || nv > n || k < 1 || k > 8 || grid < 1 || grid > kMaxPartialBlocks || step < 0 || nb_rz < 0 || nb_rz > kMaxPartialBlocks ||
        !r || !p || !dinv || (nv > 0 && !z) || !part_even || !part_odd || !scal48 || !p_flat || !p_row || !scal_flat || !scal_row)
        return REMO_ERR_ARG;
    if (uint64_t(n) * uint64_t(k) * 8 >= 0xFFFFF000ull) return fail(ctx, REMO_ERR_ARG, "remo_debug_direction_forms: n k sizeof(double) must stay below 4 GB (the flat form's range)");
    try {
        HIP_TRY(hipSetDevice(ctx->device));
        const size_t N = size_t(n) * k, NV = size_t(nv) * k, NP = size_t(nb_rz > 0 ? nb_rz : 1) * k;
        DeviceTemp tmp;
        double *dr = tmp.alloc<double>(N), *dz = tmp.alloc<double>(NV + 2), *dd = tmp.alloc<double>(n), *dpart = tmp.alloc<double>(2 * NP),
               *dscal = tmp.alloc<double>(48);
        float *dp = tmp.alloc<float>(N);
        HIP_TRY(hipMemcpy(dr, r, sizeof(double) * N, hipMemcpyHostToDevice));
        if (NV) HIP_TRY(hipMemcpy(dz, z, sizeof(double) * NV, hipMemcpyHostToDevice));
        HIP_TRY(hipMemcpy(dd, dinv, sizeof(double) * n, hipMemcpyHostToDevice));
        if (nb_rz > 0) {
            HIP_TRY(hipMemcpy(dpart, part_even, sizeof(double) * NP, hipMemcpyHostToDevice));
            HIP_TRY(hipMemcpy(dpart + NP, part_odd, sizeof(double) * NP, hipMemcpyHostToDevice));
        }
        for (int form = 1; form >= 0; --form) {
            HIP_TRY(hipMemcpy(dp, p, sizeof(float) * N, hipMemcpyHostToDevice));
            HIP_TRY(hipMemcpy(dscal, scal48, sizeof(double) * 48, hipMemcpyHostToDevice));
            launch_direction_form(form != 0, grid, n, nv, k, step, tol2, nb_rz, dpart + ((step + 1) & 1) * NP, dscal, dr, dp, dd, dz, ctx->stream);
            HIP_TRY(hipGetLastError());
            HIP_TRY(hipStreamSynchronize(ctx->stream));
            HIP_TRY(hipMemcpy(form ? p_flat : p_row, dp, sizeof(float) * N, hipMemcpyDeviceToHost));
            HIP_TRY(hipMemcpy(form ? scal_flat : scal_row, dscal, sizeof(double) * 48, hipMemcpyDeviceToHost));
        }
        return REMO_OK;
    } catch (const std::exception &ex) {
        return fail(ctx, REMO_ERR_DEVICE, ex.what());
    }
}

int remo_debug_product(remo_ctx_t *ctx, int32_t slots, int64_t cap, int64_t nx, const int32_t *xrp, const int32_t *xc, const double *xv,
                       int64_t ny, const int32_t *yrp, const int32_t *yc, const double *yv, int32_t *crp, int32_t *cc, double *cv,
                       int32_t *flags) {
    if (!ctx || !xrp || !xc || !xv || !yrp || !yc || !yv || !crp || !cc || !cv || !flags) return REMO_ERR_ARG;
    try {
        HIP_TRY(hipSetDevice(ctx->device));
        amg_debug_product(ctx->stream, slots, cap, nx, xrp, xc, xv, ny, yrp, yc, yv, crp, cc, cv, flags);
        return REMO_OK;
    } catch (const std::exception &ex) {
        return fail(ctx, REMO_ERR_DEVICE, ex.what());
    }
}

#ifdef REMO_PROBES
namespace {
long long *g_vec_stamp_buf = nullptr;
}
#endif

int remo_debug_vector_heads(remo_ctx_t *ctx, int32_t on, double *out8) {
    if (!ctx || (!on && !out8)) return REMO_ERR_ARG;
#ifndef REMO_PROBES
    return fail(ctx, REMO_ERR_ARG, "remo_debug_vector_heads: the library was built without -DREMO_PROBES (make -C remo3d_amd/csrc probes)");
#else
    const size_t words = size_t(2) * kMaxPartialBlocks * 4;
    try {
        HIP_TRY(hipSetDevice(ctx->device));
        HIP_TRY(hipStreamSynchronize(ctx->stream));
        if (on) {
            if (!g_vec_stamp_buf) HIP_TRY(hipMalloc(reinterpret_cast<void **>(&g_vec_stamp_buf), sizeof(long long) * words));
            HIP_TRY(hipMemset(g_vec_stamp_buf, 0, sizeof(long long) * words));
            set_vector_stamps(g_vec_stamp_buf);
            return REMO_OK;
        }
        set_vector_stamps(nullptr);
        for (int i = 0; i < 8; ++i) out8[i] = 0.0;
        if (!g_vec_stamp_buf) return REMO_OK;
        std::vector<long long> h(words);
        HIP_TRY(hipMemcpy(h.data(), g_vec_stamp_buf, sizeof(long long) * words, hipMemcpyDeviceToHost));
        HIP_TRY(hipFree(g_vec_stamp_buf));
        g_vec_stamp_buf = nullptr;
        for (int which = 0; which < 2; ++which) {
            double head = 0, whole = 0, share = 0, cnt = 0;
            for (int w = 0; w < kMaxPartialBlocks; ++w) {
                const long long *s4 = h.data() + (size_t(which) * kMaxPartialBlocks + w) * 4;
                if (s4[0] == 0 || s4[2] <= s4[0]) continue;
                head += double(s4[1] - s4[0]); whole += double(s4[2] - s4[0]);
                share += double(s4[1] - s4[0]) / double(s4[2] - s4[0]);
                cnt += 1;
            }
            const double c = cnt > 0 ? cnt : 1;
            out8[4 * which] = head / c; out8[4 * which + 1] = whole / c; out8[4 * which + 2] = share / c; out8[4 * which + 3] = cnt;
        }
        return REMO_OK;
    } catch (const std::exception &ex) {
        return fail(ctx, REMO_ERR_DEVICE, ex.what());
    }
#endif
}

namespace {
struct TuneKey {
    int key;
    int Tune::*field;
    int (*stored)(int) = nullptr;
};
const TuneKey kTuneKeys[] = {
    {3, &Tune::spmm_mapping},
    {6, &Tune::square},
    {9, &Tune::fold_first},
    {13, &Tune::compact},
    {15, &Tune::chain32},
    {16, &Tune::amg},
    {17, &Tune::amg32},
    {18, &Tune::element_order},
    {22, &Tune::defer_q},
    {24, &Tune::ell},
    {25, &Tune::x_in_direction},
    {29, &Tune::slab_masked},
    {30, &Tune::flat_direction},
    {31, &Tune::tile_update},
    {39, &Tune::x_ev},
    {40, &Tune::patch_rounds, [](int v) { return v == 1 ? 1 : 2; }},
    {41, &Tune::p32},
    {42, &Tune::pairs_fused},
    {43, &Tune::pair_ev_bytes},
#ifdef REMO_PROBES
    {0, &Tune::spmm_variant},
    {1, &Tune::spmm_lpr},
    {2, &Tune::spmm_threads},
    {4, &Tune::spmm_grid},
    {5, &Tune::spmm_mode},
    {7, &Tune::sq_lanes},
    {8, &Tune::row_pattern},
    {21, &Tune::patch_mode},
    {26, &Tune::patch_lean},
    {27, &Tune::slab_ahead},
    {28, &Tune::dot_bins},
    {32, &Tune::patch_spread},
    {33, &Tune::patch_trim},
    {34, &Tune::patch_persist, [](int v) { return (v == 1 || v == 2) ? v : 0; }},
    {35, &Tune::patch_wgs_per_xcd, [](int v) { return v > 0 ? v : 0; }},
    {36, &Tune::extra_apply},
#endif
};
}

int remo_debug_tune(int32_t key, int32_t value) {
    for (const TuneKey &t : kTuneKeys)
        if (t.key == key) {
            g_tune.*t.field = t.stored ? t.stored(value) : value;
            return 0;
        }
    return -1;
}

int remo_debug_sens_timing(remo_ctx_t *ctx, double *out2) {
    if (!ctx || !out2) return REMO_ERR_ARG;
    out2[0] = ctx->sens_ms;
    out2[1] = ctx->sens_bytes;
    return REMO_OK;
}

int remo_debug_sens_group_timing(remo_ctx_t *ctx, double *out4) {
    if (!ctx || !out4) return REMO_ERR_ARG;
    for (int i = 0; i < 4; ++i) out4[i] = ctx->sens_group_ms[i];
    return REMO_OK;
}

int remo_debug_field_timing(remo_ctx_t *ctx, double *out2) {
    if (!ctx || !out2) return REMO_ERR_ARG;
    out2[0] = ctx->field_ms[0];
    out2[1] = ctx->field_ms[1];
    return REMO_OK;
}

int remo_debug_pairs_timing(remo_ctx_t *ctx, double *out2) {
    if (!ctx || !out2) return REMO_ERR_ARG;
    out2[0] = ctx->pair_ms[0];
    out2[1] = ctx->pair_ms[1];
    return REMO_OK;
}

int remo_debug_pair_groups_timing(remo_ctx_t *ctx, double *out4) {
    if (!ctx || !out4) return REMO_ERR_ARG;
    for (int i = 0; i < 4; ++i) out4[i] = ctx->pair_group_ms[i];
    return REMO_OK;
}

int remo_debug_point_location(remo_ctx_t *ctx) { return ctx ? ctx->point_location : REMO_ERR_ARG; }
int remo_debug_direction_bytes(remo_ctx_t *ctx) { return ctx ? ctx->direction_bytes : REMO_ERR_ARG; }
int remo_debug_secondary_timing(remo_ctx_t *ctx, double *ms) {
    if (!ctx || !ms) return REMO_ERR_ARG;
    *ms = ctx->sec_ms;
    return REMO_OK;
}

}
```

remo3d_amd/csrc/tune.h:

```cpp
#pragma once

namespace remo {

struct Tune {
    int spmm_variant = 0;
    int spmm_lpr = 0;
    int spmm_threads = 0;
    int spmm_mapping = -1;
    int spmm_grid = 0;
    int spmm_mode = 0;
    int square = 1;
    int sq_lanes = 0;
    int row_pattern = 1;
    int fold_first = 1;
    int compact = 1;
    int chain32 = 1;
    int amg = 0;
    int amg32 = 1;
    int element_order = 1;
    int defer_q = 1;
    int ell = 1;
    int x_in_direction = 1;
    int slab_ahead = 1;
    int dot_bins = 1;
    int slab_masked = 1;
    int flat_direction = 1;
    int tile_update = 1;
    int patch_spread = 4;
    int patch_trim = 1;
    int x_ev = 1;
    int patch_rounds = 2;
    int p32 = 1;
    int pairs_fused = 1;
    int pair_ev_bytes = 0;
#ifdef REMO_PROBES
    int patch_mode = 0;
    int patch_lean = -1;
    int patch_persist = 0;
    int patch_wgs_per_xcd = 0;
    int extra_apply = 0;
#endif
};
extern Tune g_tune;

}
```

remo3d_amd/csrc/vertex_solver.hip:

```cpp
#include "vertex_solver.h"

#include <limits.h>

#include <algorithm>
#include <cmath>
#include <cstring>

#include "remo_internal.h"
#include "kutil.h"

namespace remo {

template <class T, class TC, int K, bool FIRST, int LAST, bool ELL = false>
__global__ void __launch_bounds__(256) k_cheb_step(int64_t nv, const int32_t *__restrict__ rowptr, const int32_t *__restrict__ col,
                                                   const TC *__restrict__ val, const TC *__restrict__ dinv,
                                                   const TC *__restrict__ d_old, TC *__restrict__ d_new,
                                                   TC *__restrict__ zc, TC *__restrict__ res, T *__restrict__ z, double c1_, double c2_, double inv_theta_,
                                                   T *__restrict__ r, double *__restrict__ part, const double *__restrict__ scal, int commit, int step,
                                                   const int32_t *__restrict__ ecol = nullptr, const TC *__restrict__ eval = nullptr) {
    const TC c1 = TC(c1_), c2 = TC(c2_), inv_theta = TC(inv_theta_);
    constexpr int LPR = 8, RPB = 256 / LPR;
    constexpr bool SAME = sizeof(T) == sizeof(TC);
    static_assert(K <= LPR, "one column per lane after the transposing reduction");
    if (solve_done(scal, step)) return;
    const int sub = threadIdx.x % LPR, grp = threadIdx.x / LPR;
    int idx[K], own[K];
    towner_init<K, LPR>(idx, own, sub);
    const int mycol = idx[0];
    const bool mine = own[0] != 0;
    double dot = 0.0;
    for (int64_t row = int64_t(blockIdx.x) * RPB + grp; row < nv; row += int64_t(gridDim.x) * RPB) {
        constexpr int NE = ELL ? kEllWidth / LPR : 1;
        int32_t ej[NE];
        TC ev[NE];
        int32_t rs, re;
        if constexpr (ELL) {
            const int64_t eb = row * kEllWidth + sub;
#pragma unroll
            for (int u = 0; u < NE; ++u) { ej[u] = ecol[eb + u * LPR]; ev[u] = eval[eb + u * LPR]; }
            rs = rowptr[2 * row]; re = rowptr[2 * row + 1];
        } else {
            rs = rowptr[row]; re = rowptr[row + 1];
        }
        const int64_t at = row * K + mycol;
        TC di = TC(0), dold_in = TC(0), z_in = TC(0), res_in = TC(0);
        T rr = T(0);
        if (mine) {
            di = dinv[row];
            if (SAME && commit) {
                rr = T(d_new[at]);
                r[at] = rr;
            } else {
                rr = r[at];
            }
            if (!FIRST) { dold_in = d_old[at]; z_in = zc[at]; res_in = res[at]; }
        }
        TC t[K];
#pragma unroll
        for (int c = 0; c < K; ++c) t[c] = TC(0);
        if constexpr (ELL) {
#pragma unroll
            for (int u = 0; u < NE; ++u) {
                const int32_t j = ej[u];
                const TC v = FIRST ? ev[u] * dinv[j] * inv_theta : ev[u];
                if (FIRST) {
                    const T *dj = r + int64_t(j) * K;
#pragma unroll
                    for (int c = 0; c < K; ++c) t[c] += v * TC(dj[c]);
                } else {
                    const TC *dj = d_old + int64_t(j) * K;
#pragma unroll
                    for (int c = 0; c < K; ++c) t[c] += v * dj[c];
                }
            }
        }
        for (int32_t p = rs + sub; p < re; p += LPR) {
            const int32_t j = col[p];
            if (j >= nv) break;
            const TC v = FIRST ? val[p] * dinv[j] * inv_theta : val[p];
            if (FIRST) {
                const T *dj = r + int64_t(j) * K;
#pragma unroll
                for (int c = 0; c < K; ++c) t[c] += v * TC(dj[c]);
            } else {
                const TC *dj = d_old + int64_t(j) * K;
#pragma unroll
                for (int c = 0; c < K; ++c) t[c] += v * dj[c];
            }
        }
        TReduce<K, LPR>::run(t, sub);
        if (mine) {
            const TC dold = FIRST ? di * TC(rr) * inv_theta : dold_in;
            TC zi = FIRST ? dold : z_in + dold;
            const TC ri = (FIRST ? TC(rr) : res_in) - t[0];
            const TC dn = c1 * dold + c2 * di * ri;
            if (LAST == 2) zi += dn;
            if (LAST) z[at] = T(zi / di);
            else {
                zc[at] = zi;
                res[at] = ri;
                d_new[at] = dn;
            }
            if (LAST) dot += double(rr) * double(zi);
        }
    }
    if (LAST) {
        __shared__ double smem[16 * K];
        double dcol[K];
#pragma unroll
        for (int c = 0; c < K; ++c) dcol[c] = (mine && c == mycol) ? dot : 0.0;
        block_sum<K>(dcol, smem);
#pragma unroll
        for (int c = 0; c < K; ++c)
            if (threadIdx.x == c) part[blockIdx.x * K + c] = dcol[c];
    }
}

template <class T, int K, int LPR, bool FIRST, bool LAST>
__global__ void __launch_bounds__(256) k_cheb_pair(int64_t nv, const int32_t *__restrict__ rowptr, const int32_t *__restrict__ col,
                                                   const T *__restrict__ va, const T *__restrict__ vb, const T *__restrict__ dinv,
                                                   const T *__restrict__ w_old, T *__restrict__ w_new, T *__restrict__ z, double ab_sum_, double ab_prod_,
                                                   const T *__restrict__ r, double *__restrict__ part, const double *__restrict__ scal, int step) {
    constexpr int RPB = 256 / LPR, U = 2;
    static_assert(K <= LPR, "one column per lane after the transposing reduction");
    if (solve_done(scal, step)) return;
    const T ab_sum = T(ab_sum_), ab_prod = T(ab_prod_);
    const int sub = threadIdx.x % LPR, grp = threadIdx.x / LPR;
    int idx[K], own[K];
    towner_init<K, LPR>(idx, own, sub);
    const int mycol = idx[0];
    const bool mine = own[0] != 0;
    double dot = 0.0;
    for (int64_t row = int64_t(blockIdx.x) * RPB + grp; row < nv; row += int64_t(gridDim.x) * RPB) {
        const int32_t rs = rowptr[row], re = rowptr[row + 1];
        const int64_t at = row * K + mycol;
        T di = T(0), wi = T(0), zi = T(0), rr = T(0);
        if (mine) {
            di = dinv[row];
            if (FIRST || LAST) rr = r[at];
            wi = FIRST ? di * rr : w_old[at];
            if (!FIRST) zi = z[at];
        }
        T t1[K], t2[K];
#pragma unroll
        for (int c = 0; c < K; ++c) { t1[c] = T(0); t2[c] = T(0); }
        for (int32_t p0 = rs + sub; p0 < re; p0 += U * LPR) {
            int32_t j[U];
            T a[U], b[U], w[U][K];
#pragma unroll
            for (int u = 0; u < U; ++u) {
                const int32_t p = p0 + u * LPR;
                j[u] = -1; a[u] = T(0); b[u] = T(0);
                if (p < re) { j[u] = col[p]; a[u] = va[p]; b[u] = vb[p]; }
            }
#pragma unroll
            for (int u = 0; u < U; ++u) {
#pragma unroll
                for (int c = 0; c < K; ++c) w[u][c] = T(0);
                if (j[u] >= 0) {
                    const T *wj = (FIRST ? r : w_old) + int64_t(j[u]) * K;
                    const T dj = FIRST ? dinv[j[u]] : T(1);
#pragma unroll
                    for (int c = 0; c < K; ++c) w[u][c] = FIRST ? dj * wj[c] : wj[c];
                }
            }
#pragma unroll
            for (int u = 0; u < U; ++u)
#pragma unroll
                for (int c = 0; c < K; ++c) { t1[c] += a[u] * w[u][c]; t2[c] += b[u] * w[u][c]; }
        }
        TReduce<K, LPR>::run(t1, sub);
        TReduce<K, LPR>::run(t2, sub);
        if (mine) {
            const T zn = zi + ab_sum * wi - ab_prod * di * t1[0];
            z[at] = LAST ? zn / di : zn;
            if (!LAST) w_new[at] = wi - ab_sum * di * t1[0] + ab_prod * di * t2[0];
            if (LAST) dot += double(rr) * double(zn);
        }
    }
    if (LAST) {
        __shared__ double smem[16 * K];
        double dcol[K];
#pragma unroll
        for (int c = 0; c < K; ++c) dcol[c] = (mine && c == mycol) ? dot : 0.0;
        block_sum<K>(dcol, smem);
#pragma unroll
        for (int c = 0; c < K; ++c)
            if (threadIdx.x == c) part[blockIdx.x * K + c] = dcol[c];
    }
}

int cheb_grid(int64_t nv) { return nv <= 0 ? 0 : int(std::min<int64_t>((nv + 31) / 32, kMaxPartialBlocks / 2)); }

template <class T> void launch_vertex_solve(const VertexSolverT<T> &v, int k, int step, T *r, const T *dinv, double *rz0, int nb_vec, double *part_slot,
                                            hipStream_t s, bool first_done) {
    if (v.degree <= 0 || v.nv <= 0) return;
    double *part = part_slot + int64_t(nb_vec) * k;
    if (v.amg) {
        if constexpr (sizeof(T) == 8)
            if (v.amg32) return launch_amg_cycle<float, double>(*v.amg32, k, step, (const double *)r, v.z, part, cheb_grid(v.nv), (const double *)rz0, s);
        return launch_amg_cycle<T, T>(*v.amg, k, step, (const T *)r, v.z, part, cheb_grid(v.nv), (const double *)rz0, s);
    }
    const double theta = 0.5 * (v.lmax + v.lmin), delta = 0.5 * (v.lmax - v.lmin);
    if (vertex_paired(v)) {
        const int m = v.degree, np = m / 2;
        const int g_last = cheb_grid(v.nv);
        for (int j = 0; j < np; ++j) {
            const double r1 = theta - delta * cos(M_PI * (2.0 * (j + 1) - 1.0) / (2.0 * m));
            const double r2 = theta - delta * cos(M_PI * (2.0 * (m - j) - 1.0) / (2.0 * m));
            const double a = 1.0 / r1, bb = 1.0 / r2;
            const bool first = (j == 0), last = (j + 1 == np);
            auto grid_for = [&](int lpr) { int64_t gg = (v.nv + 256 / lpr - 1) / (256 / lpr); if (last && gg > g_last) gg = g_last; if (gg > 4096) gg = 4096; return int(gg); };
            auto for_lanes = [&](auto fn) {
                if (v.sq_lanes >= 32) fn(int_c<32>{});
                else if (v.sq_lanes >= 16) fn(int_c<16>{});
                else fn(int_c<8>{});
            };
            for_k(k, [&](auto kc) { for_lanes([&](auto lc) { for_bool(first, [&](auto fc) { for_bool(last, [&](auto ec) {
                constexpr int K = decltype(kc)::value, LPR = decltype(lc)::value;
                launch256(k_cheb_pair<T, K, LPR, decltype(fc)::value, decltype(ec)::value>, grid_for(LPR), s, v.nv, v.sq_rowptr, v.sq_col, v.sq_a,
                          v.sq_b, dinv, (const T *)v.d[j & 1], v.d[(j + 1) & 1], v.z, a + bb, a * bb, r, part, rz0, step);
            }); }); }); });
        }
        return;
    }
    const double inv_theta = 1.0 / theta;
    const int g = cheb_grid(v.nv);
    const int launches = v.degree > 1 ? v.degree - 1 : 1;
    const bool chain32 = vertex_chain32(v, first_done), ell = vertex_ell(v, chain32);
    ChebStep cs{};
    for (int j = 0; j < launches; ++j) {
        cs = cheb_step(v, j == 0 ? nullptr : &cs);
        const bool first = (j == 0), last = (j + 1 == launches);
        if (first && first_done) continue;
        const int commit = (first_done && j == 1) ? 1 : 0;
        const int64_t g_rows = (v.nv + 31) / 32;
        const int gl = last ? g : int(g_rows < 8192 ? g_rows : 8192);
        auto go = [&](auto fc, auto lc) {
            for_k(k, [&](auto kc) { for_bool(ell, [&](auto ec) {
                constexpr int K = decltype(kc)::value, LAST = decltype(lc)::value;
                constexpr bool FIRST = decltype(fc)::value, ELL = decltype(ec)::value;
                if (chain32)
                    launch256(k_cheb_step<T, float, K, FIRST, LAST, ELL>, gl, s, v.nv, ELL ? v.ell_tail : v.rowptr, v.col, v.val32, v.dinv32,
                              (const float *)v.d32[j & 1], v.d32[(j + 1) & 1], v.z32, v.res32, v.z, cs.c1, cs.c2, inv_theta, r, part, rz0, 0, step,
                              v.ell_col, v.ell_val32);
                else
                    launch256(k_cheb_step<T, T, K, FIRST, LAST, ELL>, gl, s, v.nv, ELL ? v.ell_tail : v.rowptr, v.col, v.val, dinv, (const T *)v.d[j & 1], v.d[(j + 1) & 1],
                              v.z, v.res, v.z, cs.c1, cs.c2, inv_theta, r, part, rz0, commit, step, v.ell_col, v.ell_val);
            }); });
        };
        if (first && last) { if (v.degree == 1) go(std::true_type{}, int_c<1>{}); else go(std::true_type{}, int_c<2>{}); }
        else if (first) go(std::true_type{}, int_c<0>{});
        else if (last) go(std::false_type{}, int_c<2>{});
        else go(std::false_type{}, int_c<0>{});
    }
}
template void launch_vertex_solve<double>(const VertexSolverT<double> &, int, int, double *, const double *, double *, int, double *, hipStream_t, bool);
template void launch_vertex_solve<float>(const VertexSolverT<float> &, int, int, float *, const float *, double *, int, double *, hipStream_t, bool);

__global__ void __launch_bounds__(256) k_vblock_bound(int64_t nv, const int32_t *__restrict__ rowptr, const int32_t *__restrict__ col,
                                                      const double *__restrict__ val, const double *__restrict__ dinv,
                                                      unsigned long long *out_bits) {
    double m = 0.0;
    for (int64_t row = int64_t(blockIdx.x) * blockDim.x + threadIdx.x; row < nv; row += int64_t(gridDim.x) * blockDim.x) {
        double s = 0.0;
        for (int32_t p = rowptr[row]; p < rowptr[row + 1]; ++p) {
            if (col[p] >= nv) break;
            s += fabs(val[p]);
        }
        m = fmax(m, s * dinv[row]);
    }
#pragma unroll
    for (int off = 32; off > 0; off >>= 1) m = fmax(m, __shfl_xor(m, off, 64));
    if ((threadIdx.x & 63) == 0) atomicMax(out_bits, (unsigned long long)__double_as_longlong(m));
}

void launch_vblock_bound(int64_t nv, const CsrView &A, const double *dinv, unsigned long long *out_bits, hipStream_t s) {
    const int64_t g = std::clamp<int64_t>((nv + 255) / 256, 1, 512);
    hipLaunchKernelGGL(k_vblock_bound, dim3(int(g)), dim3(256), 0, s, nv, A.rowptr, A.col, A.val, dinv, out_bits);
}


template <int PASS>
__global__ void __launch_bounds__(256) k_vblock_square(int64_t nv, const int32_t *__restrict__ rowptr, const int32_t *__restrict__ col,
                                                       const double *__restrict__ val, const double *__restrict__ dinv,
                                                       int32_t *__restrict__ cnt, const int32_t *__restrict__ sq_rowptr,
                                                       int32_t *__restrict__ sq_col, double *__restrict__ sq_a, double *__restrict__ sq_b,
                                                       int64_t capacity, int32_t *flag) {
    __shared__ int32_t keys[4][kSquareSlots];
    const int wave = threadIdx.x >> 6, lane = threadIdx.x & 63;
    const int64_t row = int64_t(blockIdx.x) * 4 + wave;
    const bool active = row < nv;
    int32_t *K = keys[wave];
    for (int sl = lane; sl < kSquareSlots; sl += 64) K[sl] = INT_MAX;
    __syncthreads();
    int32_t rs = 0, re = 0;
    bool overflow = false;
    if (active) {
        rs = rowptr[row]; re = rowptr[row + 1];
        for (int32_t p = rs; p < re; ++p) {
            const int32_t k = col[p];
            if (k >= nv) break;
            const int32_t ke = rowptr[k + 1];
            for (int32_t q = rowptr[k] + lane; q < ke; q += 64) {
                const int32_t j = col[q];
                if (j >= nv) break;
                uint32_t h = (uint32_t(j) * 2654435761u) >> 23;
                bool placed = false;
                for (int probe = 0; probe < kSquareSlots; ++probe) {
                    const int32_t old = atomicCAS(&K[h], INT_MAX, j);
                    if (old == INT_MAX || old == j) { placed = true; break; }
                    h = (h + 1) & (kSquareSlots - 1);
                }
                overflow |= !placed;
            }
        }
    }
    __syncthreads();
    int c = 0;
    for (int sl = lane; sl < kSquareSlots; sl += 64) c += K[sl] != INT_MAX;
#pragma unroll
    for (int off = 32; off > 0; off >>= 1) c += __shfl_xor(c, off, 64);
    if (__builtin_amdgcn_ballot_w64(overflow) != 0 || c > kSquareSlots - 64) {
        if (lane == 0) atomicOr(flag, 1);
        c = 0;
    }
    if (PASS == 0) {
        if (active && lane == 0) cnt[row] = c;
        return;
    }
    for (int size = 2; size <= kSquareSlots; size <<= 1)
        for (int stride = size >> 1; stride > 0; stride >>= 1) {
            __syncthreads();
            for (int t = lane; t < kSquareSlots / 2; t += 64) {
                const int lo = 2 * t - (t & (stride - 1));
                const int hi = lo + stride;
                const bool up = (lo & size) == 0;
                const int32_t a = K[lo], b = K[hi];
                if ((a > b) == up) { K[lo] = b; K[hi] = a; }
            }
        }
    __syncthreads();
    if (!active || c == 0) return;
    const int64_t off = sq_rowptr[row];
    if (off + c > capacity) {
        if (lane == 0) atomicOr(flag, 2);
        return;
    }
    for (int t = lane; t < c; t += 64) {
        const int32_t j = K[t];
        double a = 0.0, b = 0.0;
        for (int32_t p = rs; p < re; ++p) {
            const int32_t k = col[p];
            if (k >= nv) break;
            if (k == j) a = val[p];
            const int32_t ks = rowptr[k], ke = rowptr[k + 1];
            const int32_t q = lower_bound_i32(col, ks, ke, j);
            if (q < ke && col[q] == j) b += val[p] * dinv[k] * val[q];
        }
        sq_col[off + t] = j;
        sq_a[off + t] = a;
        sq_b[off + t] = b;
    }
}

__global__ void __launch_bounds__(1024) k_scan_counts(int64_t n, const int32_t *__restrict__ cnt, int32_t *__restrict__ out) {
    __shared__ int64_t part[1024];
    const int64_t chunk = (n + 1023) / 1024;
    const int64_t b = int64_t(threadIdx.x) * chunk, e = (b + chunk < n) ? b + chunk : n;
    int64_t sum = 0;
    for (int64_t i = b; i < e; ++i) sum += cnt[i];
    part[threadIdx.x] = sum;
    __syncthreads();
    if (threadIdx.x == 0) {
        int64_t run = 0;
        for (int t = 0; t < 1024; ++t) { const int64_t v = part[t]; part[t] = run; run += v; }
        out[n] = int32_t(run < INT_MAX ? run : INT_MAX);
    }
    __syncthreads();
    int64_t run = part[threadIdx.x];
    for (int64_t i = b; i < e; ++i) { out[i] = int32_t(run < INT_MAX ? run : INT_MAX); run += cnt[i]; }
}

void launch_vblock_square(int64_t nv, const CsrView &A, const double *dinv, int32_t *sq_rowptr, int32_t *sq_col, double *sq_a, double *sq_b,
                          int64_t capacity, int32_t *flag, hipStream_t s) {
    if (nv <= 0) return;
    const int g = int((nv + 3) / 4);
    int32_t *cnt = sq_col;
    hipLaunchKernelGGL((k_vblock_square<0>), dim3(g), dim3(256), 0, s, nv, A.rowptr, A.col, A.val, dinv, cnt, (const int32_t *)nullptr, (int32_t *)nullptr,
                       (double *)nullptr, (double *)nullptr, capacity, flag);
    hipLaunchKernelGGL(k_scan_counts, dim3(1), dim3(1024), 0, s, nv, cnt, sq_rowptr);
    hipLaunchKernelGGL((k_vblock_square<1>), dim3(g), dim3(256), 0, s, nv, A.rowptr, A.col, A.val, dinv, (int32_t *)nullptr, sq_rowptr, sq_col, sq_a, sq_b,
                       capacity, flag);
}

template <int PASS>
__global__ void __launch_bounds__(256) k_vblock_compact(int64_t nv, const int32_t *__restrict__ rowptr, const int32_t *__restrict__ col,
                                                        const double *__restrict__ val, int32_t *__restrict__ cnt,
                                                        const int32_t *__restrict__ vb_rowptr, int32_t *__restrict__ vb_col,
                                                        double *__restrict__ vb_val, int64_t capacity, int32_t *flag) {
    const int64_t row = int64_t(blockIdx.x) * blockDim.x + threadIdx.x;
    if (row >= nv) return;
    const int32_t rs = rowptr[row], re = rowptr[row + 1];
    if (PASS == 0) {
        cnt[row] = lower_bound_i32(col, rs, re, int32_t(nv)) - rs;
    } else {
        const int32_t at = vb_rowptr[row], len = vb_rowptr[row + 1] - at;
        if (int64_t(at) + len > capacity) { if (len > 0) atomicOr(flag, 1); return; }
        for (int32_t e = 0; e < len; ++e) { vb_col[at + e] = col[rs + e]; vb_val[at + e] = val[rs + e]; }
    }
}

void launch_vblock_compact(int64_t nv, const CsrView &A, int32_t *vb_rowptr, int32_t *vb_col, double *vb_val, int64_t capacity, int32_t *flag,
                           hipStream_t s) {
    if (nv <= 0) return;
    const int g = int((nv + 255) / 256);
    int32_t *cnt = vb_col;
    hipLaunchKernelGGL((k_vblock_compact<0>), dim3(g), dim3(256), 0, s, nv, A.rowptr, A.col, A.val, cnt, (const int32_t *)nullptr, (int32_t *)nullptr,
                       (double *)nullptr, capacity, flag);
    hipLaunchKernelGGL(k_scan_counts, dim3(1), dim3(1024), 0, s, nv, cnt, vb_rowptr);
    hipLaunchKernelGGL((k_vblock_compact<1>), dim3(g), dim3(256), 0, s, nv, A.rowptr, A.col, A.val, (int32_t *)nullptr, vb_rowptr, vb_col, vb_val,
                       capacity, flag);
}

__global__ void __launch_bounds__(256) k_vblock_ell(int64_t nv, const int32_t *__restrict__ rowptr, const int32_t *__restrict__ col,
                                                    const double *__restrict__ val, int32_t *__restrict__ ecol, int32_t *__restrict__ tail,
                                                    double *__restrict__ eval64, float *__restrict__ eval32) {
    const int64_t i = int64_t(blockIdx.x) * blockDim.x + threadIdx.x;
    if (i >= nv * kEllWidth) return;
    const int64_t row = i / kEllWidth;
    const int e = int(i - row * kEllWidth);
    const int32_t rs = rowptr[row], re = rowptr[row + 1];
    int32_t c = int32_t(row);
    double v = 0.0;
    if (rs + e < re) {
        const int32_t j = col[rs + e];
        if (j < nv) { c = j; v = val[rs + e]; }
    }
    ecol[i] = c;
    if (eval64) eval64[i] = v;
    if (eval32) eval32[i] = float(v);
    if (e == 0) {
        const int32_t end = lower_bound_i32(col, rs, re, int32_t(nv));
        const bool more = end - rs > kEllWidth;
        tail[2 * row] = more ? rs + kEllWidth : 0;
        tail[2 * row + 1] = more ? end : 0;
    }
}

void launch_vblock_ell(int64_t nv, const int32_t *rowptr, const int32_t *col, const double *val, int32_t *ecol, int32_t *tail, double *eval64,
                       float *eval32, hipStream_t s) {
    if (nv <= 0) return;
    hipLaunchKernelGGL(k_vblock_ell, dim3(int((nv * kEllWidth + 255) / 256)), dim3(256), 0, s, nv, rowptr, col, val, ecol, tail, eval64, eval32);
}

static std::pair<int, double> cheb_defaults(int dim, int64_t nvfree) {
    const double nv_rel = double(nvfree > 0 ? nvfree : 1) / 12600.0;
    const double nv2 = double(nvfree > 0 ? nvfree : 1) / 25000.0;
    const int deg2 = 2 * int(std::min(16.0, std::max(8.0, std::floor(8.0 * std::sqrt(nv2) + 0.5))));
    int deg3 = int(std::min(16.0, std::max(5.0, std::floor(5.0 * std::sqrt(nv_rel) + 0.9))));
    if (deg3 > 8) deg3 &= ~1;
    if (dim == 3) return {deg3, std::min(1200.0, std::max(60.0, 90.0 * std::pow(nv_rel, 2.0 / 3.0)))};
    return {deg2, std::min(2400.0, std::max(600.0, 600.0 * nv2 * 1.25))};
}

constexpr int64_t kCompactPerRow = 48;

size_t VertexSolverBuilder::arena_bytes(int dim, int64_t nv, size_t kmax, bool want_amg, bool mixed) {
    size_t need = size_t(nv + 64) * 8 * 4 * kmax;
    need += size_t(nv + 64) * 200 * 20 + size_t(nv + 64) * 8;
    need += size_t(nv + 64) * kCompactPerRow * 16 + size_t(nv + 64) * 8;
    need += size_t(nv + 64) * kEllWidth * 12 + size_t(nv + 64) * 8;
    need += size_t(nv + 64) * (4 * 4 * kmax + 8);
    if (want_amg) need += size_t(nv + 64) * (dim == 2 ? 1536 : 3072) * 2 + (1 << 20);
    if (mixed) need += size_t(nv + 64) * 200 * 8 + size_t(nv + 64) * 4 * 4 * kmax + (1 << 16);
    return need;
}

void VertexSolverBuilder::take(Arena &ar, const VertexSolverInput &in, VertexSolverT<double> &vs) {
    two_level = (in.o.preconditioner != 0) && in.nvfree > 0;
    vs.nv = two_level ? in.nvfree : 0;
    const auto [degree, ratio] = cheb_defaults(in.dim, in.nvfree);
    ratio_default = ratio;
    vs.degree = two_level ? (in.o.coarse_degree > 0 ? in.o.coarse_degree : degree) : 0;
    nc = size_t(vs.nv) * in.kmax + 2;
    vs.z = ar.lo<double>(nc); vs.res = ar.lo<double>(nc);
    vs.d[0] = ar.lo<double>(nc); vs.d[1] = ar.lo<double>(nc);
    d_bound = ar.lo<unsigned long long>(2);
}

void VertexSolverBuilder::enqueue(Arena &ar, hipStream_t s, const VertexSolverInput &in, const CsrView &A, const double *dinv, VertexSolverT<double> &vs) {
    want_square = two_level && !in.want_amg && (vs.degree % 2 == 0) && ((g_tune.square == 1 && in.dim == 2) || g_tune.square == 2);
    want_compact = !in.lite && two_level && !want_square && (g_tune.compact == 2 || (g_tune.compact == 1 && vs.nv > 16384));
    const int64_t nvc = vs.nv;
    auto read_back = [&](const int32_t *d_flag, const int32_t *rowptr, int32_t (&h)[2]) {
        HIP_TRY(hipMemcpyAsync(&h[0], d_flag, sizeof(int32_t), hipMemcpyDeviceToHost, s));
        HIP_TRY(hipMemcpyAsync(&h[1], rowptr + nvc, sizeof(int32_t), hipMemcpyDeviceToHost, s));
    };
    if (two_level) {
        HIP_TRY(hipMemsetAsync(d_bound, 0, sizeof(unsigned long long), s));
        launch_vblock_bound(nvc, A, dinv, d_bound, s);
        HIP_TRY(hipMemcpyAsync(&h_bound, d_bound, sizeof(unsigned long long), hipMemcpyDeviceToHost, s));
    }
    if (want_square) {
        const int64_t cap = nvc * 200;
        int32_t *rowptr = ar.lo<int32_t>(size_t(nvc) + 2), *col = ar.lo<int32_t>(size_t(cap));
        double *a = ar.lo<double>(size_t(cap)), *b = ar.lo<double>(size_t(cap));
        int32_t *d_flag = ar.lo<int32_t>(1);
        HIP_TRY(hipMemsetAsync(d_flag, 0, sizeof(int32_t), s));
        launch_vblock_square(nvc, A, dinv, rowptr, col, a, b, cap, d_flag, s);
        read_back(d_flag, rowptr, h_sq);
        vs.sq_rowptr = rowptr; vs.sq_col = col; vs.sq_a = a; vs.sq_b = b;
    }
    if (want_compact) {
        const int64_t cap = (nvc + 64) * kCompactPerRow;
        int32_t *rowptr = ar.lo<int32_t>(size_t(nvc) + 2), *col = ar.lo<int32_t>(size_t(cap));
        double *val = ar.lo<double>(size_t(cap));
        int32_t *d_flag = ar.lo<int32_t>(1);
        HIP_TRY(hipMemsetAsync(d_flag, 0, sizeof(int32_t), s));
        launch_vblock_compact(nvc, A, rowptr, col, val, cap, d_flag, s);
        read_back(d_flag, rowptr, h_vb);
        vs.rowptr = rowptr; vs.col = col; vs.val = val;
    }
}

int VertexSolverBuilder::accept(Arena &ar, hipStream_t s, const VertexSolverInput &in, const CsrView &A, const double *dinv, AmgT<double> &amg64,
                                AmgT<float> &amg32, VertexSolverT<double> &vs, int *coarse_used, std::string &why) {
    const bool copied = want_compact && h_vb[0] == 0 && h_vb[1] > 0;
    if (two_level && !copied) { vs.rowptr = A.rowptr; vs.col = A.col; vs.val = A.val; }
    if (in.lite && two_level) { h_vb[0] = 0; h_vb[1] = int32_t(A.nnz); }
    vs.compact = copied || (in.lite && two_level);
    if (g_tune.chain32 && in.o.precision == 0 && vs.compact && (vs.nv > 32768 || g_tune.chain32 == 2)) {
        float *v32c = ar.lo<float>(size_t(h_vb[1]) + 4), *d32c = ar.lo<float>(size_t(vs.nv) + 4);
        launch_to_float(h_vb[1], vs.val, v32c, s);
        launch_to_float(vs.nv, dinv, d32c, s);
        vs.val32 = v32c; vs.dinv32 = d32c;
        vs.z32 = ar.lo<float>(nc); vs.res32 = ar.lo<float>(nc);
        vs.d32[0] = ar.lo<float>(nc); vs.d32[1] = ar.lo<float>(nc);
    }
    if (g_tune.ell && two_level && !in.want_amg && !want_square && in.dim == 3) {
        const size_t cells = size_t(vs.nv) * kEllWidth + 8;
        int32_t *ell_col = ar.lo<int32_t>(cells), *ell_tail = ar.lo<int32_t>(size_t(vs.nv) * 2 + 8);
        double *e64 = (in.o.precision == 0 && !vs.val32) ? ar.lo<double>(cells) : nullptr;
        float *e32 = (in.o.precision != 0 || vs.val32) ? ar.lo<float>(cells) : nullptr;
        launch_vblock_ell(vs.nv, vs.rowptr, vs.col, vs.val, ell_col, ell_tail, e64, e32, s);
        vs.ell_col = ell_col; vs.ell_tail = ell_tail; vs.ell_val = e64; vs.ell_val32 = e32;
    }
    if (two_level && in.want_amg) {
        std::string reason;
        if (amg_setup(ar, s, in.dim, vs.nv, A.rowptr, A.col, A.val, in.kmax, amg64, reason)) vs.amg = &amg64;
        else if (in.o.coarse == 2 || g_tune.amg == 2) { why = "multigrid hierarchy of the vertex block: " + reason; return REMO_ERR_NUMERIC; }
    }
    if (vs.amg && (in.o.precision == 1 || g_tune.amg32)) {
        amg_to_float(ar, s, amg64, in.kmax, amg32);
        amg32_ready = true;
        if (in.o.precision == 0) vs.amg32 = &amg32;
    }
    *coarse_used = !two_level ? 0 : (vs.amg ? 2 : 1);
    if (two_level) {
        double lmax;
        std::memcpy(&lmax, &h_bound, sizeof lmax);
        if (!(lmax > 0.0) || !std::isfinite(lmax)) { why = "vertex block has no positive spectrum bound"; return REMO_ERR_NUMERIC; }
        vs.lmax = lmax;
        vs.lmin = lmax / (in.o.coarse_ratio > 0 ? double(in.o.coarse_ratio) : ratio_default);
    }
    if (want_square && h_sq[0] != 0) vs.sq_rowptr = nullptr;
    if (vs.sq_rowptr) {
        const double avg = double(h_sq[1]) / double(vs.nv > 0 ? vs.nv : 1);
        vs.sq_lanes = g_tune.sq_lanes ? g_tune.sq_lanes : (avg > 40.0 ? 32 : (avg > 24.0 ? 16 : 8));
    }
    return REMO_OK;
}

VertexSolverT<float> VertexSolverBuilder::to_float(Arena &ar, hipStream_t s, const VertexSolverT<double> &vs, const float *val32, const AmgT<float> &amg32) const {
    VertexSolverT<float> f;
    f.nv = vs.nv; f.degree = vs.degree; f.lmax = vs.lmax; f.lmin = vs.lmin;
    f.z = ar.lo<float>(nc); f.res = ar.lo<float>(nc);
    f.d[0] = ar.lo<float>(nc); f.d[1] = ar.lo<float>(nc);
    if (vs.amg && amg32_ready) f.amg = &amg32;
    f.rowptr = vs.rowptr; f.col = vs.col; f.val = val32; f.compact = vs.compact;
    if (vs.compact) {
        float *vb32 = ar.lo<float>(size_t(h_vb[1]) + 1);
        launch_to_float(h_vb[1], vs.val, vb32, s);
        f.val = vb32;
    }
    f.ell_col = vs.ell_col; f.ell_tail = vs.ell_tail; f.ell_val = vs.ell_val32;
    if (vs.sq_rowptr) {
        float *a32 = ar.lo<float>(size_t(h_sq[1]) + 1), *b32 = ar.lo<float>(size_t(h_sq[1]) + 1);
        launch_to_float(h_sq[1], vs.sq_a, a32, s);
        launch_to_float(h_sq[1], vs.sq_b, b32, s);
        f.sq_rowptr = vs.sq_rowptr; f.sq_col = vs.sq_col; f.sq_a = a32; f.sq_b = b32; f.sq_lanes = vs.sq_lanes;
    }
    return f;
}

}
```

Baseline: 193.2.

## Add ELL image for AMG level-0 post-smoother and adaptive restriction lane widths

Builds an ELL-format copy of the finest AMG level matrix in 3D and uses a new post-smoothing kernel that processes four row groups per iteration. This batches the column/value loads before the x gathers to raise memory-level parallelism. It also picks restriction lanes-per-row from a row-length histogram so long restriction rows get wider lanes, and converts several multiply-adds to fma. The cost is extra arena memory for the ELL image, more kernel template instantiations, and a new debug entry point.

```diff
diff --git a/include/remo3d_hip_debug.h b/include/remo3d_hip_debug.h
--- a/include/remo3d_hip_debug.h
+++ b/include/remo3d_hip_debug.h
@@ -31,6 +31,9 @@
 int remo_debug_product(remo_ctx_t *ctx, int32_t slots, int64_t cap, int64_t nx, const int32_t *xrp, const int32_t *xc, const double *xv,
                        int64_t ny, const int32_t *yrp, const int32_t *yc, const double *yv, int32_t *crp, int32_t *cc, double *cv,
                        int32_t *flags);
+int remo_debug_row_ops(remo_ctx_t *ctx, int32_t op, int32_t lanes, int32_t reading, int32_t fp32, int64_t n, int64_t nx, int32_t k, const int32_t *rowptr,
+                       const int32_t *col, const double *val, const double *dinv, double omega, const double *x, const double *r, int32_t nblocks,
+                       int32_t guard, void *out, void *out2);
 int remo_debug_vector_heads(remo_ctx_t *ctx, int32_t on, double *out8);
 int remo_debug_secondary_timing(remo_ctx_t *ctx, double *ms);
 int remo_debug_pairs_timing(remo_ctx_t *ctx, double *out2);
diff --git a/remo3d_amd/_lib.py b/remo3d_amd/_lib.py
--- a/remo3d_amd/_lib.py
+++ b/remo3d_amd/_lib.py
@@ -82,7 +82,7 @@
            "remo_host_element_matrix", "remo_host_element_matrix_tensor", "remo_host_sens_element", "remo_host_factor_error", "remo_host_symbolic",
            "remo_solve_job", "remo_batch_create_job", "remo_host_point_shapes", "remo_host_secondary_element", "remo_host_error_facet", "remo_host_pair_element"]
 DEBUG_EXPORTS = ["remo_debug_stream", "remo_debug_clock", "remo_debug_device", "remo_debug_cache_gather", "remo_debug_xcc", "remo_debug_tune", "remo_debug_patch_phases", "remo_debug_patch_phases_p", "remo_debug_grid_barrier", "remo_debug_sens_timing", "remo_debug_sens_group_timing", "remo_debug_field_timing", "remo_debug_point_location", "remo_debug_secondary_timing", "remo_debug_direction_bytes", "remo_debug_pairs_timing", "remo_debug_pair_groups_timing",
-                 "remo_debug_direction_forms", "remo_debug_vector_heads", "remo_debug_product"]
+                 "remo_debug_direction_forms", "remo_debug_vector_heads", "remo_debug_product", "remo_debug_row_ops"]
 
 JOB_HEAD = ["n_mat", "sigma", "n_rhs", "src_ptr", "src_p", "src_I", "eval_ptr", "eval_p"]
 _SENS = ["u_out", "n_fun", "fun_rhs", "fun_ptr", "fun_p", "fun_w"]
@@ -219,6 +219,10 @@
     if hasattr(L, "remo_debug_product"):
         L.remo_debug_product.restype = C.c_int
         L.remo_debug_product.argtypes = [vp, C.c_int32, C.c_int64, C.c_int64, ip, ip, dp, C.c_int64, ip, ip, dp, ip, ip, dp, ip]
+    if hasattr(L, "remo_debug_row_ops"):
+        L.remo_debug_row_ops.restype = C.c_int
+        L.remo_debug_row_ops.argtypes = [vp, C.c_int32, C.c_int32, C.c_int32, C.c_int32, C.c_int64, C.c_int64, C.c_int32, ip, ip, dp, dp, C.c_double, dp, dp,
+                                         C.c_int32, C.c_int32, vp, vp]
     _lib = L
     return L
 
diff --git a/remo3d_amd/csrc/amg.h b/remo3d_amd/csrc/amg.h
--- a/remo3d_amd/csrc/amg.h
+++ b/remo3d_amd/csrc/amg.h
@@ -13,6 +13,7 @@
 
 template <class T> struct AmgLevelT {
     int64_t n = 0, nnz = 0, nnz_p = 0;
+    int r_lanes = 8;
     const int32_t *rowptr = nullptr, *col = nullptr;
     const T *val = nullptr, *dinv = nullptr;
     const int32_t *p_rowptr = nullptr, *p_col = nullptr;
@@ -20,6 +21,8 @@
     const int32_t *r_rowptr = nullptr, *r_col = nullptr;
     const T *r_val = nullptr;
     double omega = 0.0;
+    const int32_t *ell_col = nullptr, *ell_tail = nullptr;
+    const T *ell_val = nullptr;
     T *r = nullptr, *z = nullptr, *z2 = nullptr, *t = nullptr;
 };
 
@@ -35,6 +38,11 @@
                AmgT<double> &out, std::string &why);
 void amg_to_float(Arena &ar, hipStream_t s, const AmgT<double> &in, int kmax, AmgT<float> &out);
 
+void amg_level0_image(Arena &ar, hipStream_t s, AmgT<double> &h64, bool want64, AmgT<float> *h32);
+
+void amg_debug_row_ops(hipStream_t s, int op, int lanes, bool ell, bool fp32, int64_t n, int64_t nx, int k, const int32_t *rowptr, const int32_t *col,
+                       const double *val, const double *dinv, double omega, const double *x, const double *r, int nblocks, int guard, void *out, void *out2);
+
 void amg_debug_product(hipStream_t s, int slots, int64_t cap, int64_t nx, const int32_t *xrp, const int32_t *xc, const double *xv, int64_t ny,
                        const int32_t *yrp, const int32_t *yc, const double *yv, int32_t *crp, int32_t *cc, double *cv, int32_t *flags);
 
diff --git a/remo3d_amd/csrc/amg.hip b/remo3d_amd/csrc/amg.hip
--- a/remo3d_amd/csrc/amg.hip
+++ b/remo3d_amd/csrc/amg.hip
@@ -3,6 +3,7 @@
 
 #include <rocprim/device/device_scan.hpp>
 
+#include <algorithm>
 #include <atomic>
 #include <cmath>
 #include <cstdio>
@@ -350,6 +351,21 @@
     for (int t = lane; t < len; t += 64) { rc[rs + t] = K[t]; rv[rs + t] = V[t]; }
 }
 
+__global__ void __launch_bounds__(256) k_row_classes(int64_t n, const int32_t *__restrict__ rowptr, int32_t *__restrict__ over) {
+    const int64_t i = int64_t(blockIdx.x) * blockDim.x + threadIdx.x;
+    const int32_t len = i < n ? rowptr[i + 1] - rowptr[i] : 0;
+#pragma unroll
+    for (int c = 0; c < 3; ++c) {
+        const int cnt = __builtin_popcountll(__builtin_amdgcn_ballot_w64(len > (16 << c)));
+        if ((threadIdx.x & 63) == 0 && cnt) atomicAdd(&over[c], cnt);
+    }
+}
+int lanes_for_rows(int64_t rows, const int32_t *over) {
+    for (int c = 0; c < 3; ++c)
+        if (int64_t(over[c]) * 20 <= rows) return 8 << c;
+    return 64;
+}
+
 __global__ void __launch_bounds__(256) k_dense_inverse(int n, const int32_t *__restrict__ rowptr, const int32_t *__restrict__ col,
                                                        const double *__restrict__ val, double *__restrict__ inv, int32_t *flag) {
     __shared__ double a[kAmgDenseMax * kAmgDenseMax];
@@ -414,9 +430,59 @@
 #pragma unroll
         for (int u = 0; u < 2; ++u)
 #pragma unroll
-            for (int c = 0; c < K; ++c) acc[c] += a[u] * xv[u][c];
+            for (int c = 0; c < K; ++c) acc[c] = fma(a[u], xv[u][c], acc[c]);
     }
     TReduce<K, LPR>::run(acc, sub);
+}
+
+struct EllRow {
+    int32_t j[kEllWidth / kLpr];
+    int32_t rs, re;
+};
+template <class T> __device__ __forceinline__ EllRow ell_request(const AmgLevelT<T> &a, int64_t row, int sub, T (&v)[kEllWidth / kLpr]) {
+    EllRow e;
+    const int64_t eb = row * kEllWidth + sub;
+#pragma unroll
+    for (int u = 0; u < kEllWidth / kLpr; ++u) { e.j[u] = a.ell_col[eb + u * kLpr]; v[u] = a.ell_val[eb + u * kLpr]; }
+    e.rs = a.ell_tail[2 * row]; e.re = a.ell_tail[2 * row + 1];
+    return e;
+}
+template <class T, int K, bool SCALE, class TX>
+__device__ __forceinline__ void ell_gather(const AmgLevelT<T> &a, const EllRow &e, T (&v)[kEllWidth / kLpr], const TX *__restrict__ x,
+                                           T (&xv)[kEllWidth / kLpr][K]) {
+#pragma unroll
+    for (int u = 0; u < kEllWidth / kLpr; ++u) {
+        if (SCALE) v[u] *= a.dinv[e.j[u]];
+        const TX *xr = x + int64_t(e.j[u]) * K;
+#pragma unroll
+        for (int c = 0; c < K; ++c) xv[u][c] = T(xr[c]);
+    }
+}
+template <class T, int K, bool SCALE, class TX>
+__device__ __forceinline__ void ell_sum(const AmgLevelT<T> &a, const EllRow &e, const T (&v)[kEllWidth / kLpr], const T (&xv)[kEllWidth / kLpr][K], int sub,
+                                        const TX *__restrict__ x, T (&acc)[K]) {
+#pragma unroll
+    for (int c = 0; c < K; ++c) acc[c] = T(0);
+#pragma unroll
+    for (int u = 0; u < kEllWidth / kLpr; ++u)
+#pragma unroll
+        for (int c = 0; c < K; ++c) acc[c] = fma(v[u], xv[u][c], acc[c]);
+    for (int32_t p = e.rs + sub; p < e.re; p += kLpr) {
+        const int32_t j = a.col[p];
+        T av = a.val[p];
+        if (SCALE) av *= a.dinv[j];
+        const TX *xr = x + int64_t(j) * K;
+#pragma unroll
+        for (int c = 0; c < K; ++c) acc[c] = fma(av, T(xr[c]), acc[c]);
+    }
+    TReduce<K, kLpr>::run(acc, sub);
+}
+template <class T, int K, bool SCALE, class TX>
+__device__ __forceinline__ void row_product_ell(const AmgLevelT<T> &a, int64_t row, int sub, const TX *__restrict__ x, T (&acc)[K]) {
+    T v[kEllWidth / kLpr], xv[kEllWidth / kLpr][K];
+    const EllRow e = ell_request<T>(a, row, sub, v);
+    ell_gather<T, K, SCALE, TX>(a, e, v, x, xv);
+    ell_sum<T, K, SCALE, TX>(a, e, v, xv, sub, x, acc);
 }
 
 struct Lane {
@@ -440,7 +506,7 @@
         const int64_t at = row * K + ln.mycol;
         const T w = T(a.omega), ri = T(r[at]);
         a.z[at] = w * a.dinv[row] * ri;
-        a.t[at] = ri - w * acc[0];
+        a.t[at] = fma(-w, acc[0], ri);
     }
 }
 template <class T, int K, int LPR = kLpr> __device__ __forceinline__ void op_restrict(const AmgLevelT<T> &a, T *__restrict__ rn, int64_t row, const Lane &ln) {
@@ -453,18 +519,18 @@
     row_product<T, K, false>(a.p_rowptr[row], a.p_rowptr[row + 1], ln.sub, a.p_col, a.p_val, (const T *)nullptr, zn, acc);
     if (ln.mine) a.z[row * K + ln.mycol] += acc[0];
 }
-template <class T, int K, bool LAST, class TR = T>
-__device__ __forceinline__ double op_post(const AmgLevelT<T> &a, const TR *__restrict__ r, TR *__restrict__ zout, int64_t row, const Lane &ln) {
+template <class T, int K, bool LAST, class TR = T, bool ELL = false>
+__device__ __forceinline__ double op_post(const AmgLevelT<T> &a, const TR *__restrict__ r, TR *__restrict__ zout, int64_t row, const Lane &ln, double dot = 0.0) {
     T acc[K];
-    row_product<T, K, false>(a.rowptr[row], a.rowptr[row + 1], ln.sub, a.col, a.val, (const T *)nullptr, (const T *)a.z, acc);
-    double dot = 0.0;
+    if constexpr (ELL) row_product_ell<T, K, false, T>(a, row, ln.sub, (const T *)a.z, acc);
+    else row_product<T, K, false>(a.rowptr[row], a.rowptr[row + 1], ln.sub, a.col, a.val, (const T *)nullptr, (const T *)a.z, acc);
     if (ln.mine) {
         const int64_t at = row * K + ln.mycol;
         const TR rr = r[at];
         const T ri = T(rr), di = a.dinv[row];
-        const T zn = a.z[at] + T(a.omega) * di * (ri - acc[0]);
+        const T zn = fma(T(a.omega) * di, ri - acc[0], a.z[at]);
         zout[at] = TR(LAST ? zn / di : zn);
-        dot = double(rr) * double(zn);
+        dot = fma(double(rr), double(zn), dot);
     }
     return dot;
 }
@@ -478,12 +544,12 @@
     const int64_t row = int64_t(blockIdx.x) * kRpb + threadIdx.x / kLpr;
     if (row < a.n) op_pre<T, K, TR>(a, r, row, ln);
 }
-template <class T, int K>
+template <class T, int K, int LPR>
 __global__ void __launch_bounds__(256) k_amg_restrict(AmgLevelT<T> a, int64_t n_next, T *__restrict__ rn, const double *scal, int step) {
     if (amg_done(scal, step)) return;
-    const Lane ln = lane_of<K>(threadIdx.x);
-    const int64_t row = int64_t(blockIdx.x) * kRpb + threadIdx.x / kLpr;
-    if (row < n_next) op_restrict<T, K>(a, rn, row, ln);
+    const Lane ln = lane_of<K, LPR>(threadIdx.x);
+    const int64_t row = int64_t(blockIdx.x) * (256 / LPR) + threadIdx.x / LPR;
+    if (row < n_next) op_restrict<T, K, LPR>(a, rn, row, ln);
 }
 template <class T, int K>
 __global__ void __launch_bounds__(256) k_amg_prolong(AmgLevelT<T> a, const T *__restrict__ zn, const double *scal, int step) {
@@ -492,7 +558,22 @@
     const int64_t row = int64_t(blockIdx.x) * kRpb + threadIdx.x / kLpr;
     if (row < a.n) op_prolong<T, K>(a, zn, row, ln);
 }
-template <class T, int K, bool LAST, int THREADS, class TR>
+template <int K, int NW> __device__ __forceinline__ void post_partials(const Lane &ln, double dot, double *__restrict__ part) {
+    __shared__ double smem[NW * K];
+    const int lane = threadIdx.x & 63, wave = threadIdx.x >> 6;
+#pragma unroll
+    for (int k = 0; k < K; ++k) {
+        const double x = wave_sum((ln.mine && k == ln.mycol) ? dot : 0.0);
+        if (lane == 0) smem[wave * K + k] = x;
+    }
+    __syncthreads();
+    if (threadIdx.x < K) {
+        double t = 0.0;
+        for (int w = 0; w < NW; ++w) t += smem[w * K + threadIdx.x];
+        part[blockIdx.x * K + threadIdx.x] = t;
+    }
+}
+template <class T, int K, bool LAST, int THREADS, class TR, bool ELL = false>
 __global__ void __launch_bounds__(THREADS) k_amg_post(AmgLevelT<T> a, const TR *__restrict__ r, TR *__restrict__ zout,
                                                      double *__restrict__ part, const double *scal, int step) {
     if (amg_done(scal, step)) return;
@@ -500,23 +581,47 @@
     constexpr int RPB = THREADS / kLpr;
     double dot = 0.0;
     for (int64_t row = int64_t(blockIdx.x) * RPB + threadIdx.x / kLpr; row < a.n; row += int64_t(gridDim.x) * RPB)
-        dot += op_post<T, K, LAST, TR>(a, r, zout, row, ln);
-    if (LAST) {
-        constexpr int NW = THREADS / 64;
-        __shared__ double smem[NW * K];
-        const int lane = threadIdx.x & 63, wave = threadIdx.x >> 6;
-#pragma unroll
-        for (int k = 0; k < K; ++k) {
-            const double x = wave_sum((ln.mine && k == ln.mycol) ? dot : 0.0);
-            if (lane == 0) smem[wave * K + k] = x;
-        }
-        __syncthreads();
-        if (threadIdx.x < K) {
-            double t = 0.0;
-            for (int w = 0; w < NW; ++w) t += smem[w * K + threadIdx.x];
-            part[blockIdx.x * K + threadIdx.x] = t;
-        }
-    }
+        dot = op_post<T, K, LAST, TR, ELL>(a, r, zout, row, ln, dot);
+    if (LAST) post_partials<K, THREADS / 64>(ln, dot, part);
+}
+
+constexpr int kPostGroups = 4, kPostRows = kPostGroups * kRpb;
+template <class T, int K, class TR>
+__global__ void __launch_bounds__(256) k_amg_post_image(AmgLevelT<T> a, const TR *__restrict__ r, TR *__restrict__ zout, double *__restrict__ part,
+                                                        const double *scal, int step) {
+    if (amg_done(scal, step)) return;
+    constexpr int NE = kEllWidth / kLpr;
+    const Lane ln = lane_of<K>(threadIdx.x);
+    double dot = 0.0;
+    for (int64_t row0 = int64_t(blockIdx.x) * kPostRows + threadIdx.x / kLpr; row0 < a.n; row0 += int64_t(gridDim.x) * kPostRows) {
+        int64_t row[kPostGroups];
+        EllRow e[kPostGroups];
+        T v[kPostGroups][NE], xv[kPostGroups][NE][K], zi[kPostGroups], di[kPostGroups];
+        TR rr[kPostGroups];
+#pragma unroll
+        for (int g = 0; g < kPostGroups; ++g) {
+            row[g] = row0 + g * kRpb < a.n ? row0 + g * kRpb : row0;
+            e[g] = ell_request<T>(a, row[g], ln.sub, v[g]);
+            rr[g] = TR(0); zi[g] = T(0); di[g] = T(1);
+            if (ln.mine) {
+                const int64_t at = row[g] * K + ln.mycol;
+                rr[g] = r[at]; zi[g] = a.z[at]; di[g] = a.dinv[row[g]];
+            }
+        }
+#pragma unroll
+        for (int g = 0; g < kPostGroups; ++g) ell_gather<T, K, false, T>(a, e[g], v[g], (const T *)a.z, xv[g]);
+#pragma unroll
+        for (int g = 0; g < kPostGroups; ++g) {
+            T acc[K];
+            ell_sum<T, K, false, T>(a, e[g], v[g], xv[g], ln.sub, (const T *)a.z, acc);
+            if (ln.mine && row0 + g * kRpb < a.n) {
+                const T zn = fma(T(a.omega) * di[g], T(rr[g]) - acc[0], zi[g]);
+                zout[row[g] * K + ln.mycol] = TR(zn / di[g]);
+                dot = fma(double(rr[g]), double(zn), dot);
+            }
+        }
+    }
+    post_partials<K, 4>(ln, dot, part);
 }
 
 template <class T, int K>
@@ -535,15 +640,15 @@
     AmgLevelT<T> lev[kTailLevels];
     const T *inv;
 };
-template <class T, int K>
+template <class T, int K, int LPR0>
 __global__ void __launch_bounds__(1024) k_amg_tail(AmgTailT<T> A, const double *scal, int step) {
     if (amg_done(scal, step)) return;
     const Lane ln = lane_of<K>(threadIdx.x);
     const int g = threadIdx.x / kLpr, ng = 1024 / kLpr;
     const int L = A.levels;
     {
-        const Lane l16 = lane_of<K, 16>(threadIdx.x);
-        for (int64_t row = threadIdx.x / 16; row < A.lev[0].n; row += 1024 / 16) op_restrict<T, K, 16>(A.up, A.lev[0].r, row, l16);
+        const Lane l0 = lane_of<K, LPR0>(threadIdx.x);
+        for (int64_t row = threadIdx.x / LPR0; row < A.lev[0].n; row += 1024 / LPR0) op_restrict<T, K, LPR0>(A.up, A.lev[0].r, row, l0);
         __syncthreads();
     }
     for (int l = 0; l + 1 < L; ++l) {
@@ -570,6 +675,21 @@
 }
 
 int grid_rows(int64_t n, int per_block) { return int((n + per_block - 1) / per_block); }
+
+template <class T> bool level_image(const AmgLevelT<T> &a) { return a.ell_col && a.ell_tail && a.ell_val; }
+template <int MIN = 8, class F> void for_lanes(int lanes, F &&fn) {
+    if (lanes >= 64) fn(int_c<64>{});
+    else if (lanes >= 32) fn(int_c<32>{});
+    else if (lanes >= 16 || MIN >= 16) fn(int_c<16>{});
+    else if constexpr (MIN < 16) fn(int_c<8>{});
+}
+#ifdef REMO_PROBES
+template <class T> int restrict_lanes(const AmgLevelT<T> &a) { return g_tune.amg_r_lanes ? g_tune.amg_r_lanes : a.r_lanes; }
+bool post_wide() { return g_tune.amg_post_wide != 0; }
+#else
+template <class T> int restrict_lanes(const AmgLevelT<T> &a) { return a.r_lanes; }
+constexpr bool post_wide() { return false; }
+#endif
 
 void scan_counts(Arena &ar, hipStream_t s, int64_t n, const int32_t *cnt, int32_t *out) {
     size_t tb = 0;
@@ -609,6 +729,31 @@
 std::atomic<int> g_product_hint[2][kAmgMaxLevels][3];
 std::atomic<int> g_ap_room[2];
 constexpr int kFlagSlots = 64;
+constexpr int kClassSlot = 32;
+static_assert(8 + 3 * kAmgMaxLevels <= kClassSlot && kClassSlot + 4 * kAmgMaxLevels <= kFlagSlots, "flag slots overlap");
+
+void print_row_lengths(hipStream_t s, const AmgT<double> &H) {
+    auto stats = [&](const char *name, int l, const int32_t *d_rowptr, int64_t n) {
+        if (!d_rowptr || n <= 0) return;
+        std::vector<int32_t> rp(size_t(n) + 1);
+        HIP_TRY(hipMemcpyAsync(rp.data(), d_rowptr, sizeof(int32_t) * rp.size(), hipMemcpyDeviceToHost, s));
+        HIP_TRY(hipStreamSynchronize(s));
+        std::vector<int32_t> len(static_cast<size_t>(n));
+        for (int64_t i = 0; i < n; ++i) len[size_t(i)] = rp[size_t(i) + 1] - rp[size_t(i)];
+        std::sort(len.begin(), len.end());
+        fprintf(stderr, "amg level %d %s: %lld rows, entries per row min %d median %d 95 %% %d max %d\n", l, name, (long long)n, len.front(),
+                len[size_t(n / 2)], len[size_t((n * 95) / 100)], len.back());
+    };
+    for (int l = 0; l < H.levels; ++l) {
+        const AmgLevelT<double> &a = H.lev[l];
+        stats("A", l, a.rowptr, a.n);
+        if (l + 1 < H.levels) {
+            stats("P", l, a.p_rowptr, a.n);
+            stats("R", l, a.r_rowptr, H.lev[l + 1].n);
+            fprintf(stderr, "amg level %d R: %d lanes per row\n", l, a.r_lanes);
+        }
+    }
+}
 
 int amg_build(Arena &ar, hipStream_t s, int hs, int64_t nv, const int32_t *rowptr, const int32_t *col, const double *val, int kmax, AmgT<double> &H,
               std::string &why) {
@@ -741,6 +886,7 @@
             hipLaunchKernelGGL(k_tr_fill, dim3(g), dim3(256), 0, s, n, P.rowptr, P.col, P.val, R.rowptr, cursor, R.col, R.val);
             hipLaunchKernelGGL((k_tr_sort<0, kTrMax, 4>), dim3(grid_rows(nc, 4)), dim3(256), 0, s, nc, R.rowptr, R.col, R.val, d_flag);
             hipLaunchKernelGGL((k_tr_sort<kTrMax, kTrMaxLong, 1>), dim3(grid_rows(nc, 1)), dim3(64), 0, s, nc, R.rowptr, R.col, R.val, d_flag);
+            hipLaunchKernelGGL(k_row_classes, dim3(grid_rows(nc, 256)), dim3(256), 0, s, nc, R.rowptr, d_flag + kClassSlot + 4 * L);
         }
         lv.r_rowptr = R.rowptr; lv.r_col = R.col; lv.r_val = R.val;
         Csr AP, Ac;
@@ -758,7 +904,11 @@
     const int verdict = check(L);
     if (verdict != 0) return verdict;
     H.lev[L].nnz = h_nnz_a[L];
-    for (int l = 0; l < L; ++l) H.lev[l].nnz_p = h_nnz_p[l];
+    for (int l = 0; l < L; ++l) {
+        H.lev[l].nnz_p = h_nnz_p[l];
+        H.lev[l].r_lanes = lanes_for_rows(H.lev[l + 1].n, h_flags + kClassSlot + 4 * l);
+    }
+    if (getenv("REMO_AMG_DEBUG")) print_row_lengths(s, H);
     H.launches = 4 * (H.levels - 1);
     H.kmax = kmax;
     return 0;
@@ -840,6 +990,109 @@
     HIP_TRY(hipStreamSynchronize(s));
 }
 
+namespace {
+template <class T>
+void debug_row_ops(hipStream_t s, int op, int lanes, bool ell, int64_t n, int64_t nx, int k, const int32_t *rowptr, const int32_t *col, const double *val,
+                   const double *dinv, double omega, const double *x, const double *r, int nblocks, int guard, void *out, void *out2) {
+    const size_t nnz = size_t(rowptr[n]), nk = size_t(n) * k, nxk = size_t(nx) * k, cells = size_t(n) * kEllWidth + 8;
+    const size_t bytes = 4 * (size_t(n) + 2 + nnz + 2 + cells + 2 * size_t(n) + 8) + 8 * (2 * nnz + 4 + size_t(n) + nxk + 4 * nk + 2 * cells) +
+                         8 * (size_t(nblocks) * k + 3 * size_t(guard)) + 256 * 32;
+    DeviceTemp tmp;
+    Arena ar;
+    ar.base = tmp.alloc<char>(bytes);
+    ar.cap = bytes;
+    HIP_TRY(hipMemsetAsync(ar.base, 0xFF, bytes, s));
+    std::vector<std::vector<char>> keep;
+    auto put = [&](auto tag, const double *src, size_t count) {
+        using D = decltype(tag);
+        D *d = ar.lo<D>(count + 2);
+        keep.emplace_back(sizeof(D) * (count + 1));
+        D *h = reinterpret_cast<D *>(keep.back().data());
+        for (size_t i = 0; i < count; ++i) h[i] = D(src[i]);
+        if (count) HIP_TRY(hipMemcpyAsync(d, h, sizeof(D) * count, hipMemcpyHostToDevice, s));
+        return d;
+    };
+    int32_t *d_rp = ar.lo<int32_t>(size_t(n) + 2), *d_col = ar.lo<int32_t>(nnz + 2);
+    HIP_TRY(hipMemcpyAsync(d_rp, rowptr, sizeof(int32_t) * (size_t(n) + 1), hipMemcpyHostToDevice, s));
+    if (nnz) HIP_TRY(hipMemcpyAsync(d_col, col, sizeof(int32_t) * nnz, hipMemcpyHostToDevice, s));
+    AmgLevelT<T> a;
+    a.n = n; a.nnz = int64_t(nnz); a.omega = omega;
+    const T *d_val = put(T(0), val, nnz);
+    a.rowptr = d_rp; a.col = d_col; a.val = d_val;
+    if (op != 0) a.dinv = put(T(0), dinv, size_t(n));
+    if (ell) {
+        const double *d_val64 = put(double(0), val, nnz);
+        int32_t *ecol = ar.lo<int32_t>(cells), *tail = ar.lo<int32_t>(size_t(n) * 2 + 8);
+        T *ev = ar.lo<T>(cells);
+        double *e64 = nullptr;
+        float *e32 = nullptr;
+        if constexpr (sizeof(T) == 8) e64 = ev; else e32 = ev;
+        launch_vblock_ell(n, d_rp, d_col, d_val64, ecol, tail, e64, e32, s);
+        a.ell_col = ecol; a.ell_tail = tail; a.ell_val = ev;
+    }
+    auto result = [&](auto tag, size_t count) { return ar.lo<decltype(tag)>(count + size_t(guard)); };
+    auto fetch = [&](void *dst, const void *src, size_t elem, size_t count) {
+        HIP_TRY(hipMemcpyAsync(dst, src, elem * (count + size_t(guard)), hipMemcpyDeviceToHost, s));
+    };
+    const double *scal = nullptr;
+    for_k(k, [&](auto kc) {
+        constexpr int K = decltype(kc)::value;
+        if (op == 0) {
+            a.r_rowptr = d_rp; a.r_col = d_col; a.r_val = d_val;
+            a.t = put(T(0), x, nxk);
+            T *rn = result(T(0), nk);
+            for_lanes(lanes, [&](auto lc) {
+                constexpr int LPR = decltype(lc)::value;
+                launch256(k_amg_restrict<T, K, LPR>, grid_rows(n, 256 / LPR), s, a, n, rn, scal, 0);
+            });
+            fetch(out, rn, sizeof(T), nk);
+        } else if (op == 1) {
+            const double *d_r = put(double(0), x, nk);
+            a.z = result(T(0), nk); a.t = result(T(0), nk);
+            launch256(k_amg_pre<T, K, double>, grid_rows(n, kRpb), s, a, d_r, scal, 0);
+            fetch(out, a.z, sizeof(T), nk);
+            fetch(out2, a.t, sizeof(T), nk);
+        } else if (op == 2) {
+            a.z = put(T(0), x, nk);
+            const T *d_r = put(T(0), r, nk);
+            T *zout = result(T(0), nk);
+            launch256(k_amg_post<T, K, false, 256, T>, grid_rows(n, kRpb), s, a, d_r, zout, (double *)nullptr, scal, 0);
+            fetch(out, zout, sizeof(T), nk);
+        } else {
+            a.z = put(T(0), x, nk);
+            const double *d_r = put(double(0), r, nk);
+            double *zout = result(double(0), nk), *part = result(double(0), size_t(nblocks) * k);
+            if (ell) launch256(k_amg_post_image<T, K, double>, nblocks, s, a, d_r, zout, part, scal, 0);
+            else hipLaunchKernelGGL((k_amg_post<T, K, true, 1024, double>), dim3(nblocks), dim3(1024), 0, s, a, d_r, zout, part, scal, 0);
+            fetch(out, zout, sizeof(double), nk);
+            fetch(out2, part, sizeof(double), size_t(nblocks) * k);
+        }
+    });
+    HIP_TRY(hipGetLastError());
+    HIP_TRY(hipStreamSynchronize(s));
+}
+}
+
+void amg_debug_row_ops(hipStream_t s, int op, int lanes, bool ell, bool fp32, int64_t n, int64_t nx, int k, const int32_t *rowptr, const int32_t *col,
+                       const double *val, const double *dinv, double omega, const double *x, const double *r, int nblocks, int guard, void *out, void *out2) {
+    if (op < 0 || op > 3) throw std::runtime_error("amg_debug_row_ops: op 0 .. 3");
+    if (lanes != 8 && lanes != 16 && lanes != 32 && lanes != 64) throw std::runtime_error("amg_debug_row_ops: 8, 16, 32 or 64 lanes");
+    if (op != 0 && lanes != 8) throw std::runtime_error("amg_debug_row_ops: the sweeps take 8 lanes per row");
+    if (ell && op != 3) throw std::runtime_error("amg_debug_row_ops: only the finest level's second half sweep (op 3) reads the fixed-width image");
+    if (n < 1 || nx < 1 || n > (1 << 22) || nx > (1 << 22) || k < 1 || k > 8 || guard < 0 || guard > 4096) throw std::runtime_error("amg_debug_row_ops: sizes out of range");
+    if (op != 0 && nx != n) throw std::runtime_error("amg_debug_row_ops: a sweep needs a square matrix");
+    if (op == 3 && (nblocks < 1 || nblocks > kMaxPartialBlocks / 2)) throw std::runtime_error("amg_debug_row_ops: workgroups out of range");
+    if (op != 3) nblocks = 0;
+    if (!x || (op != 0 && !dinv) || (op >= 2 && !r) || (op == 1 || op == 3 ? !out2 : false)) throw std::runtime_error("amg_debug_row_ops: an array is missing");
+    if (rowptr[0] != 0) throw std::runtime_error("amg_debug_row_ops: row pointers must ascend from 0");
+    for (int64_t i = 0; i < n; ++i)
+        if (rowptr[i + 1] < rowptr[i] || rowptr[i + 1] > (1 << 26)) throw std::runtime_error("amg_debug_row_ops: row pointers must ascend from 0");
+    for (int32_t p = 0; p < rowptr[n]; ++p)
+        if (col[p] < 0 || col[p] >= nx) throw std::runtime_error("amg_debug_row_ops: a column names no row of x");
+    if (fp32) debug_row_ops<float>(s, op, lanes, ell, n, nx, k, rowptr, col, val, dinv, omega, x, r, nblocks, guard, out, out2);
+    else debug_row_ops<double>(s, op, lanes, ell, n, nx, k, rowptr, col, val, dinv, omega, x, r, nblocks, guard, out, out2);
+}
+
 void amg_to_float(Arena &ar, hipStream_t s, const AmgT<double> &in, int kmax, AmgT<float> &out) {
     auto conv = [&](const double *src, size_t count) {
         float *dst = ar.lo<float>(count + 4);
@@ -860,13 +1113,25 @@
         if (l > 0) b.r = ar.lo<float>(size_t(a.n) * kmax + 4);
         if (l + 1 < in.levels) {
             b.p_rowptr = a.p_rowptr; b.p_col = a.p_col; b.r_rowptr = a.r_rowptr; b.r_col = a.r_col;
-            b.nnz_p = a.nnz_p;
+            b.nnz_p = a.nnz_p; b.r_lanes = a.r_lanes;
             b.p_val = conv(a.p_val, size_t(a.nnz_p));
             b.r_val = conv(a.r_val, size_t(a.nnz_p));
         }
     }
     const int64_t nc = in.lev[in.levels - 1].n;
     out.inv = conv(in.inv, size_t(nc * nc));
+}
+
+void amg_level0_image(Arena &ar, hipStream_t s, AmgT<double> &h64, bool want64, AmgT<float> *h32) {
+    AmgLevelT<double> &a = h64.lev[0];
+    if (h64.levels < 2 || a.n <= 0 || (!want64 && !h32)) return;
+    const size_t cells = size_t(a.n) * kEllWidth + 8;
+    int32_t *ecol = ar.lo<int32_t>(cells), *tail = ar.lo<int32_t>(size_t(a.n) * 2 + 8);
+    double *e64 = want64 ? ar.lo<double>(cells) : nullptr;
+    float *e32 = h32 ? ar.lo<float>(cells) : nullptr;
+    launch_vblock_ell(a.n, a.rowptr, a.col, a.val, ecol, tail, e64, e32, s);
+    if (want64) { a.ell_col = ecol; a.ell_tail = tail; a.ell_val = e64; }
+    if (h32) { AmgLevelT<float> &b = h32->lev[0]; b.ell_col = ecol; b.ell_tail = tail; b.ell_val = e32; }
 }
 
 template <class T, class TR> void launch_amg_cycle(const AmgT<T> &H, int k, int step, const TR *r, TR *cz, double *part, int nblocks, const double *scal, hipStream_t s) {
@@ -874,13 +1139,18 @@
     auto rows_grid = [&](int64_t n) { return int((n + kRpb - 1) / kRpb); };
     int lt = L - 1;
     while (lt > 1 && H.lev[lt - 1].n <= kTailRows && L - (lt - 1) <= kTailLevels) --lt;
+    const bool image = level_image(H.lev[0]);
     for_k(k, [&](auto kc) {
         constexpr int K = decltype(kc)::value;
         for (int l = 0; l < lt; ++l) {
             const AmgLevelT<T> &a = H.lev[l], &b = H.lev[l + 1];
-            if (l == 0) hipLaunchKernelGGL((k_amg_pre<T, K, TR>), dim3(rows_grid(a.n)), dim3(256), 0, s, a, r, scal, step);
-            else hipLaunchKernelGGL((k_amg_pre<T, K, T>), dim3(rows_grid(a.n)), dim3(256), 0, s, a, (const T *)a.r, scal, step);
-            if (l + 1 < lt) hipLaunchKernelGGL((k_amg_restrict<T, K>), dim3(rows_grid(b.n)), dim3(256), 0, s, a, b.n, b.r, scal, step);
+            if (l == 0) launch256(k_amg_pre<T, K, TR>, rows_grid(a.n), s, a, r, scal, step);
+            else launch256(k_amg_pre<T, K, T>, rows_grid(a.n), s, a, (const T *)a.r, scal, step);
+            if (l + 1 < lt)
+                for_lanes(restrict_lanes(a), [&](auto lc) {
+                    constexpr int LPR = decltype(lc)::value;
+                    launch256(k_amg_restrict<T, K, LPR>, grid_rows(b.n, 256 / LPR), s, a, b.n, b.r, scal, step);
+                });
         }
         {
             AmgTailT<T> tail;
@@ -888,13 +1158,21 @@
             tail.up = H.lev[lt - 1];
             for (int l = lt; l < L; ++l) tail.lev[l - lt] = H.lev[l];
             tail.inv = H.inv;
-            hipLaunchKernelGGL((k_amg_tail<T, K>), dim3(1), dim3(1024), 0, s, tail, scal, step);
+            for_lanes<16>(restrict_lanes(tail.up), [&](auto lc) {
+                hipLaunchKernelGGL((k_amg_tail<T, K, decltype(lc)::value>), dim3(1), dim3(1024), 0, s, tail, scal, step);
+            });
         }
         for (int l = lt - 1; l >= 0; --l) {
             const AmgLevelT<T> &a = H.lev[l], &b = H.lev[l + 1];
             hipLaunchKernelGGL((k_amg_prolong<T, K>), dim3(rows_grid(a.n)), dim3(256), 0, s, a, (const T *)b.z2, scal, step);
-            if (l == 0)
-                hipLaunchKernelGGL((k_amg_post<T, K, true, 1024, TR>), dim3(nblocks), dim3(1024), 0, s, a, r, cz, part, scal, step);
+            if (l == 0 && image && !post_wide())
+                launch256(k_amg_post_image<T, K, TR>, nblocks, s, a, r, cz, part, scal, step);
+#ifdef REMO_PROBES
+            else if (l == 0 && image)
+                hipLaunchKernelGGL((k_amg_post<T, K, true, 1024, TR, true>), dim3(nblocks), dim3(1024), 0, s, a, r, cz, part, scal, step);
+#endif
+            else if (l == 0)
+                hipLaunchKernelGGL((k_amg_post<T, K, true, 1024, TR, false>), dim3(nblocks), dim3(1024), 0, s, a, r, cz, part, scal, step);
             else
                 hipLaunchKernelGGL((k_amg_post<T, K, false, 256, T>), dim3(rows_grid(a.n)), dim3(256), 0, s, a, (const T *)a.r, a.z2, (double *)nullptr, scal, step);
         }
diff --git a/remo3d_amd/csrc/remo_debug.hip b/remo3d_amd/csrc/remo_debug.hip
--- a/remo3d_amd/csrc/remo_debug.hip
+++ b/remo3d_amd/csrc/remo_debug.hip
@@ -398,6 +398,19 @@
     try {
         HIP_TRY(hipSetDevice(ctx->device));
         amg_debug_product(ctx->stream, slots, cap, nx, xrp, xc, xv, ny, yrp, yc, yv, crp, cc, cv, flags);
+        return REMO_OK;
+    } catch (const std::exception &ex) {
+        return fail(ctx, REMO_ERR_DEVICE, ex.what());
+    }
+}
+
+int remo_debug_row_ops(remo_ctx_t *ctx, int32_t op, int32_t lanes, int32_t reading, int32_t fp32, int64_t n, int64_t nx, int32_t k, const int32_t *rowptr,
+                       const int32_t *col, const double *val, const double *dinv, double omega, const double *x, const double *r, int32_t nblocks,
+                       int32_t guard, void *out, void *out2) {
+    if (!ctx || !rowptr || !col || !val || !x || !out || (reading != 0 && reading != 1)) return REMO_ERR_ARG;
+    try {
+        HIP_TRY(hipSetDevice(ctx->device));
+        amg_debug_row_ops(ctx->stream, op, lanes, reading == 1, fp32 != 0, n, nx, k, rowptr, col, val, dinv, omega, x, r, nblocks, guard, out, out2);
         return REMO_OK;
     } catch (const std::exception &ex) {
         return fail(ctx, REMO_ERR_DEVICE, ex.what());
@@ -494,6 +507,9 @@
     {34, &Tune::patch_persist, [](int v) { return (v == 1 || v == 2) ? v : 0; }},
     {35, &Tune::patch_wgs_per_xcd, [](int v) { return v > 0 ? v : 0; }},
     {36, &Tune::extra_apply},
+    {44, &Tune::amg_r_lanes, [](int v) { return (v == 8 || v == 16 || v == 32 || v == 64) ? v : 0; }},
+    {45, &Tune::amg_image},
+    {46, &Tune::amg_post_wide},
 #endif
 };
 }
diff --git a/remo3d_amd/csrc/tune.h b/remo3d_amd/csrc/tune.h
--- a/remo3d_amd/csrc/tune.h
+++ b/remo3d_amd/csrc/tune.h
@@ -39,6 +39,9 @@
     int patch_persist = 0;
     int patch_wgs_per_xcd = 0;
     int extra_apply = 0;
+    int amg_r_lanes = 0;
+    int amg_image = 1;
+    int amg_post_wide = 0;
 #endif
 };
 extern Tune g_tune;
diff --git a/remo3d_amd/csrc/vertex_solver.hip b/remo3d_amd/csrc/vertex_solver.hip
--- a/remo3d_amd/csrc/vertex_solver.hip
+++ b/remo3d_amd/csrc/vertex_solver.hip
@@ -464,6 +464,12 @@
     return {deg2, std::min(2400.0, std::max(600.0, 600.0 * nv2 * 1.25))};
 }
 
+#ifdef REMO_PROBES
+static bool amg_wants_image() { return g_tune.amg_image != 0; }
+#else
+static constexpr bool amg_wants_image() { return true; }
+#endif
+
 constexpr int64_t kCompactPerRow = 48;
 
 size_t VertexSolverBuilder::arena_bytes(int dim, int64_t nv, size_t kmax, bool want_amg, bool mixed) {
@@ -473,6 +479,7 @@
     need += size_t(nv + 64) * kEllWidth * 12 + size_t(nv + 64) * 8;
     need += size_t(nv + 64) * (4 * 4 * kmax + 8);
     if (want_amg) need += size_t(nv + 64) * (dim == 2 ? 1536 : 3072) * 2 + (1 << 20);
+    if (want_amg && dim == 3) need += size_t(nv + 64) * kEllWidth * 16 + size_t(nv + 64) * 8;
     if (mixed) need += size_t(nv + 64) * 200 * 8 + size_t(nv + 64) * 4 * 4 * kmax + (1 << 16);
     return need;
 }
@@ -556,6 +563,7 @@
         amg32_ready = true;
         if (in.o.precision == 0) vs.amg32 = &amg32;
     }
+    if (vs.amg && in.dim == 3 && amg_wants_image()) amg_level0_image(ar, s, amg64, in.o.precision == 0 && !vs.amg32, amg32_ready ? &amg32 : nullptr);
     *coarse_used = !two_level ? 0 : (vs.amg ? 2 : 1);
     if (two_level) {
         double lmax;
```

New measurement: 200.5 (median of 6 runs). +3.7%, better.
